# stochasticHydroTools/PSE

Measured on AMD Instinct MI355X. Metric: BD particle-steps/s (full PSE Brownian step: M.F + k-space noise + Lanczos M^1/2.psi + Euler), N=1e6, phi=0.1, higher is better.
Workload: dtype f64; 1 GPU; random-sphere suspension N=1000000, phi=0.1, cubic L=347.29, grid 256^3, xi=0.4405, rcut=5.966, P=6, error=0.001, kT=1.0, dt=0.001; parallelism=1 GPU

## Files before the change

pse_amd/csrc/pse_capi.hip:

```cpp
#include <hip/hip_runtime.h>
#include <rccl/rccl.h>
#include <rocfft/rocfft.h>

#include <algorithm>
#include <chrono>
#include <cmath>
#include <cstdarg>
#include <cstdio>
#include <cstring>
#include <dlfcn.h>
#include <functional>
#include <future>
#include <memory>
#include <mutex>
#include <thread>
#include <string>
#include <vector>

#include "../../include/pse_amd.h"
#include "pse_err.h"
#include "pse_host.h"
#include "pse_kernels.h"
#include "pse_farfield.h"
#include "pse_fft.h"
// ... 637 lines not shown
        if (T->m[0]->grid_slabs > 1) *mask |= 1u << PH_COMM;
        TRY(wave_compute(*T, a, 0));
        next = 1;
        if (T->m[0]->grid_slabs == 1) return upto(1 << 30);
        return 0;
    }
    int upto(int e) {
        while (T && next <= 3 && slot[next - 1] <= e) {
            TRY(wave_exchange(*T, next - 1));
            TRY(wave_compute(*T, a, next));
            ++next;
        }
        return 0;
    }
    int drain() { return upto(1 << 30); }
};

static int row_ranges(const pse_handle *h, int N, int depth, int rg[3][2]) {
    if (h->n_slabs == 1) { rg[0][0] = 0; rg[0][1] = N; return 1; }
    const int G = h->n_slabs, r = h->slab_rank, L = (r + G - 1) % G, R = (r + 1) % G;
    int n = 0;
    auto add = [&](int a, int b) {
        if (b <= a) return;
        for (int q = 0; q < n; ++q) if (rg[q][0] == a && rg[q][1] == b) return;
        rg[n][0] = a; rg[n][1] = b; ++n;
    };
    rg[0][0] = h->row_lo[r]; rg[0][1] = h->row_lo[r + 1]; n = 1;
    if (depth >= 1) {
        add((depth == 1 ? h->last_begin : h->last2_begin)[L], h->row_lo[L + 1]);
        add(h->row_lo[R], (depth == 1 ? h->first_end : h->first2_end)[R]);
    }
    return n;
}
static RowMap rank_rows(const pse_handle *h, int N, int depth) {
    int rg[3][2];
    const int n = row_ranges(h, N, depth, rg);
    return row_map(rg, n);
}

static int real(pse_team &T, double4 *pse_handle::*vec, double4 *pse_handle::*out, size_t vec_off, size_t out_off, int N,
                bool build_list, bool with_psi = false, int depth = 0) {
    for (pse_handle *h : act(T)) {
        h->w_is_mpsi = false;
        int mode = MREAL_CELLS;
        if (h->nb.cap > 0) {
            if (h->nb_valid) mode = MREAL_USE_LIST;
            else if (build_list) mode = MREAL_BUILD_LIST;
        }
        int vlm = VL_NONE;
        if (h->vl_use) vlm = VL_USE;
        else if (h->vl_pending && mode != MREAL_USE_LIST) vlm = VL_WRITE;
        const double4 *v = h->*vec + vec_off;
        if (h->gated && mode == MREAL_CELLS) {
            const RowMap rows = rank_rows(h, N, 0);
            const int nco = h->n_intervals * 2 * RS_NCOEF;
            const Gate rb{h->gate_word, 1}, ru{h->gate_word, 0};
            launch_mreal(h->pos_s, h->posf_s, v, h->*out + out_off, rows, h->cell_off, h->dbox, h->nc, h->d.rcut, h->d.self, h->coef, nco,
                         h->nb, MREAL_CELLS, h->stream, nullptr, nullptr, h->vl, VL_WRITE, nullptr, nullptr, 0, nullptr, rb);
            launch_gate_copy(rb, h->pos_build, h->pos_s, (size_t)N, h->stream);
            launch_mreal(h->pos_s, h->posf_s, v, h->*out + out_off, rows, h->cell_off, h->dbox, h->nc, h->d.rcut, h->d.self, h->coef, nco,
                         h->nb, MREAL_CELLS, h->stream, nullptr, nullptr, h->vl, VL_USE,
                         v == h->f_s && h->pv_is_f ? h->pv : nullptr, nullptr, 0, nullptr, ru);
            h->vl_valid = true; h->vl_box = h->box;
            continue;
        }
        const bool psi = with_psi && mode == MREAL_BUILD_LIST;
        launch_mreal(h->pos_s, h->posf_s, v, h->*out + out_off, rank_rows(h, N, mode == MREAL_BUILD_LIST ? depth : 0), h->cell_off, h->dbox,
                     h->nc, h->d.rcut, h->d.self, h->coef, h->n_intervals * 2 * RS_NCOEF, h->nb, mode, h->stream,
                     psi ? h->psi_s : nullptr, h->w_s, h->vl, vlm,
                     v == h->f_s && h->pv_is_f && (vlm == VL_USE || mode != MREAL_USE_LIST) ? h->pv : nullptr,
                     psi && h->n_slabs == 1 ? h->partials : nullptr, h->npart_cap, h->scal);
        h->sums0_done = psi && h->n_slabs == 1 && vlm != VL_USE && mreal_table_in_lds(h->n_intervals * 2 * RS_NCOEF);
        if (vlm == VL_WRITE) {
            HIPCHK(hipMemcpyAsync(h->pos_build, h->pos_s, (size_t)N * sizeof(double4), hipMemcpyDeviceToDevice, h->stream));
            h->vl_pending = false; h->vl_valid = true; h->vl_box = h->box;
        }
        if (mode == MREAL_BUILD_LIST) { h->nb_valid = true; h->w_is_mpsi = with_psi && (vlm == VL_USE || mreal_table_in_lds(h->n_intervals * 2 * RS_NCOEF)); }
    }
    return 0;
}

static int update_ranges(const pse_handle *h, int N, int rg[3][2]) { return row_ranges(h, N, 1, rg); }

static double4 *lz_vec(const pse_handle *h, int q) { return q < 0 ? nullptr : q == 0 ? h->psi_s : h->V + (size_t)q * h->n_pad; }
static LzBlockArgs lz_block_args(const pse_handle *h, int j, bool full) {
    LzBlockArgs a{};
    a.q = lz_vec(h, j); a.p = lz_vec(h, j - 1); a.w1 = h->w_s; a.w2 = full ? h->w2_s : nullptr;
    a.u = h->u_s; a.v1 = lz_vec(h, j + 1); a.v2 = full ? lz_vec(h, j + 2) : nullptr;
    a.j = j;
    return a;
}
static int lz_m_in(const int *m_io) { return std::min(std::max(m_io ? *m_io : 2, 1), M_MAX); }
static int lz_queued_extra(const pse_handle *h, int m_in) {
    return std::max(0, std::min(h->lz_extra >= 0 ? h->lz_extra : h->tun.lz_extra, M_MAX - std::max(m_in, 2)));
}

static int lz_wait_scalars(pse_team &T, bool &hook_done, const std::function<int()> &before_first_wait) {
    pse_handle *h0 = T.m[0];
    HIPCHK(hipEventRecord(h0->ev_scal, h0->stream));
    if (!hook_done) {
        hook_done = true;
        for (pse_handle *h : act(T)) TRY(te(h, PH_LANCZOS));
        if (before_first_wait) TRY(before_first_wait());
    }
    HIPCHK(hipEventSynchronize(h0->ev_scal));
    return 0;
}
static int lz_decide_batch(LzDecide d, int m_in, int done, double tol, const double *sc, LzState &st) {
    d.m_lo = std::max((d.first ? 0 : st.checked) + 1, std::max(m_in - 1, 1)); d.m_hi = d.done_iters = done; d.m_max = M_MAX; d.tol = tol;
    int at = 0;
    const LzFailure f = lz_decide_host(d, sc, st, &at);
    if (f == LZ_NONFINITE) return fail(PSE_ERR_NUMERIC, "Lanczos produced a non-finite coefficient at iteration %d", at);
    if (f == LZ_EIGEN_FAILED) return fail(PSE_ERR_NUMERIC, "tridiagonal eigen-solve failed at m = %d", at);
    return 0;
}
static int lz_zero_result(pse_team &T, int N, int matvecs) {
    for (pse_handle *h : act(T)) {
        HIPCHK(hipMemsetAsync(h->ub_s, 0, (size_t)N * sizeof(double4), h->stream));
        h->info.lanczos_m = 0; h->info.lanczos_matvecs = matvecs; h->info.lanczos_stepnorm = 0.0;
    }
    return 0;
}
static void lz_combine(pse_team &T, int N, double scale, const LzState &st, int matvecs, int exchanges) {
    BasisCoef tc{};
    std::copy(st.coef, st.coef + st.m_final, tc.t);
    for (pse_handle *h : act(T)) {
        int lo, hi;
        row_range(h, N, lo, hi);
        launch_basis_combine(h->psi_s, h->V, h->n_pad, tc, st.m_final, h->scal, scale, 1, h->ub_s, lo, hi, h->stream, h->sink);
        h->tail_done = h->sink.on;
        h->info.lanczos_m = st.m_final; h->info.lanczos_matvecs = matvecs; h->info.lanczos_stepnorm = st.stepnorm;
        h->info.lanczos_exchanges = exchanges;
    }
}

static int lanczos_queued(pse_team &T, int N, double tol, double scale, int *m_io, const std::function<int()> &before_first_wait,
                          const std::function<int()> &before_combine) {
    pse_handle *h = T.m[0];
    const int m_in = lz_m_in(m_io), target = std::max(m_in, 2), extra = lz_queued_extra(h, m_in);
    const int *stop = &h->lz_state->done;
    const double seq = (double)++h->lz_seq;
    h->lz_last_queued = true;
    int rg[3][2];
    const int nrg_all = update_ranges(h, N, rg);
    auto vector_part = [&](int j, const int *gate) {
        launch_lz_update(lz_vec(h, j), h->w_s, lz_vec(h, j - 1), lz_vec(h, j + 1), j, h->scal, rg, nrg_all, h->stream,
                         nullptr, 0, h->sc_host_dev, gate, vq_of(h), h->lz_sums);
    };
    auto iteration = [&](int j, bool scalars_only, const int *gate) -> int {
        const bool have_y = j == 0 && h->w_is_mpsi;
        const bool fused = !have_y && h->nb.cap > 0 && h->nb_valid;
        if (!fused && !have_y) {
            if (gate) return fail(PSE_ERR_NUMERIC, "queued Lanczos: a gated iteration needs the pair list");
            TRY(real(T, j == 0 ? &pse_handle::psi_s : &pse_handle::V, &pse_handle::w_s, (size_t)j * h->n_pad, 0, N, true));
        }
        const double4 *vjm1 = lz_vec(h, j - 1);
        const bool split = fused && j > 0;
        if (fused)
            launch_mreal_lanczos(h->pos_s, lz_vec(h, j), h->w_s, row_map(0, N), h->cell_off, h->dbox, h->nc, h->d.rcut, h->d.self, h->coef, h->nb,
                                 LzFuse{split ? nullptr : vjm1, h->partials, h->npart_cap, nullptr, nullptr, nullptr, h->lz_sums, lz_update_grid(N)}, h->scal, nullptr, nullptr, h->stream,
                                 h->vl_use ? h->vl : VerletList{}, split ? 4 : 1, gate, DevRowArgs{}, j > 0 ? vq_of(h) : nullptr);
        else if (!(j == 0 && h->sums0_done))
            launch_lz_dots(lz_vec(h, j), h->w_s, vjm1, 0, N, h->partials, h->npart_cap, h->scal, h->stream);
        h->w_is_mpsi = false; h->sums0_done = false;
        if (scalars_only) launch_lz_update(lz_vec(h, j), h->w_s, vjm1, lz_vec(h, j + 1), j, h->scal, rg, 0, h->stream, nullptr, 0,
                                           h->sc_host_dev, gate);
        else vector_part(j, gate);
        return 0;
    };
    for (int j = 0; j < target; ++j) TRY(iteration(j, j == target - 1, nullptr));
    LzDecide d{};
    d.m_lo = std::max(m_in - 1, 1); d.m_hi = target; d.done_iters = target; d.first = 1; d.last = extra == 0 ? 1 : 0; d.m_max = M_MAX; d.tol = tol;
    launch_lz_decide(d, h->scal, h->lz_state, h->sc_host_dev, seq, h->stream);
    int done = target;
    for (int x = 0; x < extra; ++x) {
        vector_part(done - 1, stop);
        TRY(iteration(done, true, stop));
        d.m_lo = d.m_hi = done + 1; d.done_iters = done + 1; d.pending_beta = done; d.first = 0; d.last = x == extra - 1 ? 1 : 0;
        launch_lz_decide(d, h->scal, h->lz_state, h->sc_host_dev, seq, h->stream);
        ++done;
    }
    TRY(te(h, PH_LANCZOS));
    if (before_first_wait) TRY(before_first_wait());
    if (before_combine) TRY(before_combine());
    launch_basis_combine(h->psi_s, h->V, h->n_pad, BasisCoef{}, 0, h->scal, scale, 1, h->ub_s, 0, N, h->stream, h->sink, h->lz_state);
    h->tail_done = h->sink.on;
    h->info.lanczos_matvecs = done; h->info.lanczos_exchanges = 0;
    if (m_io) *m_io = h->sc_host[LZ_HOST_SEQ] > 0.0 && h->sc_host[LZ_HOST_M] >= 1.0 ? (int)h->sc_host[LZ_HOST_M] : m_in;
    HIPCHK(hipGetLastError());
    return 0;
}

static int lanczos(pse_team &T, int N, double tol, double scale, int *m_io, const std::function<int()> &before_first_wait = nullptr,
                   WavePump *pump = nullptr, const std::function<int()> &before_combine = nullptr) {
    pse_handle *h0 = T.m[0];
    const int m_in = lz_m_in(m_io);
    if (h0->async_mode && T.G == 1 && T.solo < 0 && h0->nb.cap > 0 && !h0->timing &&
        lz_decide_supported(std::max(m_in, 2) + lz_queued_extra(h0, m_in)))
        return lanczos_queued(T, N, tol, scale, m_io, before_first_wait, before_combine);
    for (pse_handle *h : act(T)) h->lz_last_queued = false;
    const double *sc = h0->sc_host;
    int done = 0, n_exchanges = 0;
    int target = std::max(m_in, 2);
    int pending_beta = 0;
    LzState st{0, 0, 0, 0, 1.0, {}, {}};
    bool hook_done = false;
    auto update = [&](int j, bool scalars_only) {
        for (pse_handle *h : act(T)) {
            int rg[3][2];
            const int nrg = scalars_only ? 0 : update_ranges(h, N, rg);
            launch_lz_update(lz_vec(h, j), h->w_s, lz_vec(h, j - 1), lz_vec(h, j + 1), j, h->scal, rg, nrg, h->stream, h->sums_all, T.G > 1 ? T.G : 0,
                             h == h0 ? h->sc_host_dev : nullptr, nullptr, T.G <= 1 ? vq_of(h) : nullptr, T.G <= 1 ? h->lz_sums : nullptr);
        }
    };
    while (true) {
        for (; done < target; ++done) {
            const bool have_y = done == 0 && h0->w_is_mpsi;
            const bool fused = !have_y && h0->nb.cap > 0 && h0->nb_valid;
            const bool timed = done == 1 && fused;
            if (!fused && !have_y) TRY(real(T, done == 0 ? &pse_handle::psi_s : &pse_handle::V, &pse_handle::w_s, (size_t)done * h0->n_pad, 0, N, true));
            for (pse_handle *h : act(T)) {
                int lo, hi;
                row_range(h, N, lo, hi);
                const double4 *xj = lz_vec(h, done), *vjm1 = lz_vec(h, done - 1);
                if (fused) {
                    const bool ev = timed && h->timing;
                    const bool split = done > 0 && T.G <= 1;
                    launch_mreal_lanczos(h->pos_s, xj, h->w_s, row_map(lo, hi), h->cell_off, h->dbox, h->nc, h->d.rcut, h->d.self, h->coef,
                                         h->nb, LzFuse{split ? nullptr : vjm1, h->partials, h->npart_cap, nullptr, nullptr, nullptr, h->lz_sums, lz_update_grid(N)}, h->scal,
                                         ev ? h->ph[PH_MATVEC].a : nullptr, ev ? h->ph[PH_MATVEC].b : nullptr, h->stream,
                                         h->vl_use ? h->vl : VerletList{}, split ? 4 : 1, nullptr, DevRowArgs{}, done > 0 && T.G <= 1 ? vq_of(h) : nullptr);
                    if (timed) h->matvec_timed = true;
                } else if (!(done == 0 && h->sums0_done)) {
                    launch_lz_dots(xj, h->w_s, vjm1, lo, hi, h->partials, h->npart_cap, h->scal, h->stream);
                }
                h->w_is_mpsi = false; h->sums0_done = false;
            }
            if (pump) TRY(pump->upto(n_exchanges));
            ++n_exchanges;
            TRY(team_lanczos_exchange(T, [](pse_handle *h) { return (double *)h->w_s; }));
            update(done, done == target - 1);
        }
        TRY(lz_wait_scalars(T, hook_done, before_first_wait));
        if (T.solo >= 0) { st.m_final = done; break; }
        LzDecide d{};
        d.first = pending_beta == 0; d.pending_beta = pending_beta;
        TRY(lz_decide_batch(d, m_in, done, tol, sc, st));
        if (st.done) break;
        update(done - 1, false);
        pending_beta = done;
        target = std::min(M_MAX, done + std::max(2, done / 4));
    }
    if (st.m_final == 0) {
        if (m_io) *m_io = m_in;
        return lz_zero_result(T, N, done);
    }
    if (before_combine) TRY(before_combine());
    lz_combine(T, N, scale, st, done, T.G > 1 ? n_exchanges : 0);
    if (m_io) *m_io = st.m_final;
    return 0;
}

static int lanczos_team(pse_team &T, int N, double tol, double scale, int *m_io, const std::function<int()> &before_first_wait,
                        WavePump *pump, const std::function<int()> &before_combine = nullptr) {
    pse_handle *h0 = T.m[0];
    for (pse_handle *h : act(T)) h->lz_last_queued = false;
    const int m_in = lz_m_in(m_io);
    const double *sc = h0->sc_host;
    int done = 0, target = std::max(m_in, 2), n_exchanges = 0, matvecs = 0;
    int half_pending = -1;
    bool first = true;
    LzState st{0, 0, 0, 0, 1.0, {}, {}};
    bool hook_done = false;
    while (true) {
        while (done < target) {
            if (half_pending >= 0) {
                for (pse_handle *h : act(T)) {
                    int rg[3][2];
                    const int nrg = row_ranges(h, N, 2, rg);
                    launch_lz_block(lz_block_args(h, half_pending, false), false, h->scal, rg, nrg, h->stream, h->sums_all, T.G, h == h0 ? h->sc_host_dev : nullptr);
                }
                half_pending = -1;
            }
            const int j = done;
            const bool full = target - done >= 2 && j + 2 <= M_MAX;
            for (pse_handle *h : act(T)) {
                const LzFuse lz{nullptr, h->partials, h->npart_cap, lz_vec(h, j), lz_vec(h, j - 1), j > 0 ? h->u_s : nullptr};
                if (j == 0 && !h->w_is_mpsi) return fail(PSE_ERR_NUMERIC, "two-step Lanczos: M psi did not come with the pair list");
                if (!(j == 0 && h->w_is_mpsi)) {
                    launch_mreal_lanczos(h->pos_s, lz_vec(h, j), h->w_s, rank_rows(h, N, full ? 1 : 0), h->cell_off, h->dbox, h->nc, h->d.rcut,
                                         h->d.self, h->coef, h->nb, lz, h->scal, nullptr, nullptr, h->stream, VerletList{}, full ? 0 : 3);
                    ++matvecs;
                } else if (!full) {
                    return fail(PSE_ERR_NUMERIC, "two-step Lanczos: a single step cannot start at j = 0");
                }
                h->w_is_mpsi = false;
                if (full) {
                    launch_mreal_lanczos(h->pos_s, h->w_s, h->w2_s, rank_rows(h, N, 0), h->cell_off, h->dbox, h->nc, h->d.rcut, h->d.self,
                                         h->coef, h->nb, lz, h->scal, nullptr, nullptr, h->stream, VerletList{}, 2);
                    ++matvecs;
                }
            }
            if (pump) TRY(pump->upto(n_exchanges));
            ++n_exchanges;
            TRY(team_run_exchange(T, [&](pse_handle *h) {
                                      auto ops = ghost_ops(h, T.G, {(double *)h->w_s, full ? (double *)h->w2_s : nullptr}, 2);
                                      sum_ops(h, T.G, LZ_NGRAM, ops);
                                      return ops; },
                                  false, DIAG_LANCZOS));
            for (pse_handle *h : act(T)) {
                int rg[3][2];
                const int nrg = full ? row_ranges(h, N, 2, rg) : 0;
                launch_lz_block(lz_block_args(h, j, full), full, h->scal, rg, nrg, h->stream, h->sums_all, T.G, h == h0 ? h->sc_host_dev : nullptr);
            }
            if (full) done += 2; else { done += 1; half_pending = j; }
        }
        TRY(lz_wait_scalars(T, hook_done, before_first_wait));
        if (T.solo >= 0) { st.m_final = done; break; }
        LzDecide d{};
        d.first = first; d.have_last_beta = d.normalised = 1;
        TRY(lz_decide_batch(d, m_in, done, tol, sc, st));
        if (st.done) break;
        first = false;
        target = std::min(M_MAX, done + std::max(2, done / 4));
    }
    if (st.m_final == 0) {
        if (m_io) *m_io = m_in;
        return lz_zero_result(T, N, matvecs);
    }
    if (half_pending >= 0 && st.m_final > half_pending + 1) return fail(PSE_ERR_NUMERIC, "two-step Lanczos: basis vector %d was never formed", half_pending + 1);
    if (before_combine) TRY(before_combine());
    lz_combine(T, N, scale, st, matvecs, n_exchanges);
    if (m_io) *m_io = st.m_final;
    return 0;
}

struct Args {
    const double4 *pos; const double4 *force; double4 *vel;
};

struct StepArgs {
    double4 *pos; double4 *vel; double3 *accel; int3 *image; const double4 *force;
};
struct StepTail { const std::vector<StepArgs> *sa; double dt, shear_rate; };

static int velocity(pse_team &T, const std::vector<Args> &a, const unsigned *group, int N, int parts, double kT, double dt,
                    unsigned timestep, int *m_io, unsigned *mask, const StepTail *tail = nullptr) {
    for (pse_handle *h : T.m)
        if (h->loc.on) return fail(PSE_ERR_INVALID, "this handle is an owned-particle rank (pse_params.local_rows): drive it through pse_team_step_local");
    for (pse_handle *h : T.m) h->tail_done = false;
    diag_begin(T);
    for (size_t r = 0; r < T.m.size(); ++r)
        if (T.solo < 0 || T.m[r]->slab_rank == T.solo)
            TRY(prepare(T.m[r], a[r].pos, a[r].force, group, N, true, false, PrepExtra{kT > 0.0, timestep}, (parts & 1) != 0));
    *mask |= 1u << PH_SORT;
    const bool noise = kT > 0.0;
    const bool sstep = T.G > 1 && noise && (parts & 1) && team_sstep(T.m[0]);
    for (pse_handle *h : act(T)) {
        const bool on = h->side && parts == 3 && !h->timing && (T.G > 1 ? T.lanes : (h->overlap_all || !noise));
        if (on != h->side_on || h->wstream != (on ? h->side : h->stream)) {
            h->side_on = on;
            h->wstream = on ? h->side : h->stream;
            TRY(bind_wave_stream(h));
        }
    }
    WavePump pump;
    const WaveArgs wa{N, noise, kT, dt, timestep};
    auto wave_start = [&]() -> int { return pump.start(T, wa, T.m[0]->tun.team_sched, mask); };
    const bool wave_behind = noise && (parts & 2) && (parts & 1) && !T.m[0]->side_on;
    const bool near_first = noise && parts == 3 && T.m[0]->side_on;
// ... 74 lines not shown
        }
        HIPCHK(hipGetLastError());
    }
    diag_mark(T, 1, act(T)[0]->stream);
    return 0;
}

static int team_of_one(pse_handle *h, pse_team &T) {
    if (h->n_slabs > 1) return fail(PSE_ERR_INVALID, "this handle is a slab rank: drive it through a pse_team");
    T.m = {h}; T.G = 1;
    return 0;
}

static int do_mobility(pse_team &T, const std::vector<Args> &a, const unsigned *group, unsigned N, int parts) {
    for (pse_handle *h : T.m) TRY(check_n(h, N));
    for (auto &x : a) if (!x.pos || !x.force || !x.vel) return fail(PSE_ERR_INVALID, "null array");
    if (!(parts & 3)) return fail(PSE_ERR_INVALID, "parts must select real (1), wave (2) or both (3)");
    unsigned mask = 1u << PH_TOTAL;
    for (pse_handle *h : act(T)) TRY(ts(h, PH_TOTAL));
    TRY(velocity(T, a, group, (int)N, parts, 0.0, 1.0, 0, nullptr, &mask));
    for (pse_handle *h : act(T)) { TRY(te(h, PH_TOTAL)); TRY(collect_times(h, mask)); }
    return 0;
}

static int do_brownian(pse_team &T, const std::vector<Args> &a, const unsigned *group, unsigned N, double kT, double dt,
                       unsigned timestep, int *lanczos_m, int parts = 3) {
    for (pse_handle *h : act(T)) TRY(check_n(h, N));
    for (auto &x : a) if (!x.pos || !x.force || !x.vel) return fail(PSE_ERR_INVALID, "null array");
    if (kT < 0 || !(dt > 0)) return fail(PSE_ERR_INVALID, "need kT >= 0 and dt > 0");
    unsigned mask = 1u << PH_TOTAL;
    for (pse_handle *h : act(T)) TRY(ts(h, PH_TOTAL));
    TRY(velocity(T, a, group, (int)N, parts, kT, dt, timestep, lanczos_m, &mask));
    for (pse_handle *h : act(T)) { TRY(te(h, PH_TOTAL)); TRY(collect_times(h, mask)); }
    return 0;
}

static int do_step(pse_team &T, const std::vector<StepArgs> &sa, const unsigned *group, unsigned N, double kT, double dt,
                   unsigned timestep, double shear_rate, int *lanczos_m) {
    for (pse_handle *h : act(T)) TRY(check_n(h, N));
    std::vector<Args> a;
    for (auto &x : sa) {
        if (!x.pos || !x.vel || !x.accel || !x.image || !x.force) return fail(PSE_ERR_INVALID, "null array");
        a.push_back(Args{x.pos, x.force, x.vel});
    }
    if (kT < 0 || !(dt > 0)) return fail(PSE_ERR_INVALID, "need kT >= 0 and dt > 0");
    unsigned mask = (1u << PH_TOTAL) | (1u << PH_INTEG);
    for (pse_handle *h : act(T)) TRY(ts(h, PH_TOTAL));
    for (pse_handle *h : act(T)) h->vl_kind = 1;
    const StepTail tail{&sa, dt, shear_rate};
    const int rc_v = velocity(T, a, group, (int)N, 3, kT, dt, timestep, lanczos_m, &mask, &tail);
    for (pse_handle *h : act(T)) h->vl_kind = 0;
    if (rc_v) return rc_v;
    for (pse_handle *h : act(T)) {
        TRY(te(h, PH_TOTAL));
        HIPCHK(hipGetLastError());
        TRY(collect_times(h, mask));
    }
    return 0;
}

static LocalRegions local_regions(const pse_handle *h) {
    const LocalGeom &g = h->loc.g;
    const int lc = layer_cells(h->nc), nx = g.nx;
    auto wrap = [&](int l) { return ((l % nx) + nx) % nx; };
    LocalRegions r{};
    const int l_own = g.rank * g.per, l_gl = wrap(l_own - g.depth), l_gr = wrap(l_own + g.per);
    r.c0[0] = l_own * lc; r.c1[0] = (l_own + g.per) * lc; r.base[0] = 0; r.cap[0] = g.c_own;
    r.c0[1] = l_gl * lc; r.c1[1] = (l_gl + g.depth) * lc; r.base[1] = g.c_own; r.cap[1] = g.c_g;
    r.c0[2] = l_gr * lc; r.c1[2] = (l_gr + g.depth) * lc; r.base[2] = g.c_own + g.c_g; r.cap[2] = g.c_g;
    r.c_first_end = (l_own + g.depth) * lc - 1;
    r.c_last_begin = (l_own + g.per - g.depth) * lc;
    r.c_gl_adj = wrap(l_own - 1) * lc;
    r.c_gr_adj = (l_gr + 1) * lc - 1;
    return r;
}

static int lanczos_local(pse_team &T, double tol, int *m_io, WavePump *pump) {
    pse_handle *h0 = T.m[0];
    const int m_in = lz_m_in(m_io), target = std::max(m_in, 2);
    const int extra_blocks = ((T.lz_extra >= 0 ? T.lz_extra : h0->tun.lz_extra) + 1) / 2;
    if (target + 2 * extra_blocks > M_MAX || !lz_decide_supported(target + 2 * extra_blocks))
        return fail(PSE_ERR_INVALID, "owned-particle step: starting count %d of the Lanczos iteration is beyond what the device-side decision takes", m_in);
    int n_exchanges = 0, matvecs = 0, done = 0, half_pending = -1;
    auto fuse = [&](pse_handle *h, int j) { return LzFuse{nullptr, h->partials, h->npart_cap, lz_vec(h, j), lz_vec(h, j - 1), j > 0 ? h->u_s : nullptr}; };
    auto exchange = [&](bool full) -> int {
        if (pump) TRY(pump->upto(n_exchanges));
        ++n_exchanges;
        return team_run_exchange(T, [&](pse_handle *h) {
            const LocalGeom &g = h->loc.g;
            const int L = (g.rank + g.G - 1) % g.G, R = (g.rank + 1) % g.G;
            const size_t cnt = (size_t)g.c_g * 4;
            std::vector<Xfer> ops;
            ops.push_back(Xfer{(double *)h->w_s, cnt, L, (double *)(h->w_s + g.c_own + g.c_g), cnt, R});
            ops.push_back(Xfer{(double *)h->loc.stage_w1, cnt, R, (double *)(h->w_s + g.c_own), cnt, L});
            if (full) {
                ops.push_back(Xfer{(double *)h->w2_s, cnt, L, (double *)(h->w2_s + g.c_own + g.c_g), cnt, R});
                ops.push_back(Xfer{(double *)h->loc.stage_w2, cnt, R, (double *)(h->w2_s + g.c_own), cnt, L});
            }
            sum_ops(h, T.G, LZ_NGRAM, ops);
            return ops; }, false, DIAG_LANCZOS);
    };
    auto full_block = [&](int j, bool gated) -> int {
        for (pse_handle *h : act(T)) {
            const int *gate = gated ? &h->lz_state->done : nullptr;
            const LocalRows *R = h->loc.rows;
            if (j == 0) {
                if (!h->w_is_mpsi) return fail(PSE_ERR_NUMERIC, "owned-particle step: M psi did not come with the pair list");
            } else {
                launch_mreal_lanczos(h->pos_s, lz_vec(h, j), h->w_s, RowMap{}, h->cell_off, h->dbox, h->nc, h->d.rcut, h->d.self, h->coef, h->nb, fuse(h, j),
                                     h->scal, nullptr, nullptr, h->stream, VerletList{}, 0, gate,
                                     DevRowArgs{&R->own1, R, h->loc.stage_w1, h->loc.rows_cap, h->loc.g.c_g});
                ++matvecs;
            }
            h->w_is_mpsi = false;
            launch_mreal_lanczos(h->pos_s, h->w_s, h->w2_s, RowMap{}, h->cell_off, h->dbox, h->nc, h->d.rcut, h->d.self, h->coef, h->nb, fuse(h, j), h->scal,
                                 nullptr, nullptr, h->stream, VerletList{}, 2, gate, DevRowArgs{&R->own, R, h->loc.stage_w2, h->loc.g.c_own, h->loc.g.c_g});
            ++matvecs;
        }
        TRY(exchange(true));
        for (pse_handle *h : act(T))
            launch_lz_block(lz_block_args(h, j, true), true, h->scal, nullptr, 0, h->stream, h->sums_all, T.G, h->sc_host_dev, &h->loc.rows->all,
                            h->loc.rows_cap, false, gated ? &h->lz_state->done : nullptr);
        return 0;
    };
    auto single = [&](int j, bool gated) -> int {
        for (pse_handle *h : act(T)) {
            const LocalRows *R = h->loc.rows;
            launch_mreal_lanczos(h->pos_s, lz_vec(h, j), h->w_s, RowMap{}, h->cell_off, h->dbox, h->nc, h->d.rcut, h->d.self, h->coef, h->nb, fuse(h, j), h->scal,
                                 nullptr, nullptr, h->stream, VerletList{}, 3, gated ? &h->lz_state->done : nullptr,
                                 DevRowArgs{&R->own, R, h->loc.stage_w1, h->loc.g.c_own, h->loc.g.c_g});
            ++matvecs;
        }
        TRY(exchange(false));
        for (pse_handle *h : act(T))
            launch_lz_block(lz_block_args(h, j, false), false, h->scal, nullptr, 0, h->stream, h->sums_all, T.G, h->sc_host_dev, &h->loc.rows->all,
                            h->loc.rows_cap, true, gated ? &h->lz_state->done : nullptr);
        half_pending = j;
        return 0;
    };
    auto decide = [&](int m_lo, int m_hi, int done_iters, bool first, bool last) {
        for (pse_handle *h : act(T)) {
            LzDecide d{};
            d.m_lo = m_lo; d.m_hi = m_hi; d.done_iters = done_iters; d.have_last_beta = 1; d.first = first ? 1 : 0; d.last = last ? 1 : 0;
            d.normalised = 1; d.m_max = M_MAX; d.tol = T.solo >= 0 ? 1e300 : tol;
            launch_lz_decide(d, h->scal, h->lz_state, h->sc_host_dev, (double)h->lz_seq, h->stream);
        }
    };
    for (pse_handle *h : act(T)) { ++h->lz_seq; h->lz_last_queued = true; }
    while (target - done >= 2) { TRY(full_block(done, false)); done += 2; }
    if (target - done == 1) { TRY(single(done, false)); done += 1; }
    decide(std::max(m_in - 1, 1), target, done, true, extra_blocks == 0);
    for (int x = 0; x < extra_blocks; ++x) {
        if (half_pending >= 0) {
            for (pse_handle *h : act(T))
                launch_lz_block(lz_block_args(h, half_pending, false), false, h->scal, nullptr, 0, h->stream, h->sums_all, T.G, h->sc_host_dev,
                                &h->loc.rows->all, h->loc.rows_cap, false, &h->lz_state->done);
            half_pending = -1;
        }
        TRY(full_block(done, true));
        decide(done + 1, done + 2, done + 2, false, x == extra_blocks - 1);
        done += 2;
    }
    for (pse_handle *h : act(T)) { h->info.lanczos_matvecs = matvecs; h->info.lanczos_exchanges = n_exchanges; }
    if (m_io) *m_io = !remote(T) && h0->sc_host[LZ_HOST_SEQ] > 0.0 && h0->sc_host[LZ_HOST_M] >= 1.0 ? (int)h0->sc_host[LZ_HOST_M] : m_in;
    return 0;
}

// ... 140 lines not shown
    if (parts < 1 || parts > 3) return fail(PSE_ERR_INVALID, "parts must select real (1), wave (2) or both (3)");
    if (!pos || !force || !vel) return fail(PSE_ERR_INVALID, "null array");
    pse_team T;
    TRY(team_of_one(h, T));
    return do_brownian(T, {Args{(const double4 *)pos, (const double4 *)force, (double4 *)vel}}, group, N, kT, dt, timestep, lanczos_m, parts);
}

extern "C" int pse_integrate(pse_handle *h, pse_double4 *pos, const pse_double4 *vel, pse_double3 *accel, pse_int3 *image,
                             const pse_double4 *net_force, const unsigned *group, unsigned N, double dt, double shear_rate) {
    if (!h) return fail(PSE_ERR_INVALID, "null handle");
    if (!pos || !vel || !accel || !image || !net_force) return fail(PSE_ERR_INVALID, "null array");
    if (!(dt > 0)) return fail(PSE_ERR_INVALID, "need dt > 0");
    TRY(check_n(h, N));
    HIPCHK(hipSetDevice(h->device));
    launch_integrate((double4 *)pos, (const double4 *)vel, (double3 *)accel, (int3 *)image, (const double4 *)net_force, group, (int)N, h->dbox, dt,
                     shear_rate, h->stream);
    HIPCHK(hipGetLastError());
    return 0;
}

extern "C" int pse_step(pse_handle *h, pse_double4 *pos, pse_double4 *vel, pse_double3 *accel, pse_int3 *image,
                        const pse_double4 *net_force, const unsigned *group, unsigned N, double kT, double dt,
                        unsigned timestep, double shear_rate, int *lanczos_m) {
    if (!h) return fail(PSE_ERR_INVALID, "null handle");
    pse_team T;
    TRY(team_of_one(h, T));
    return do_step(T, {StepArgs{(double4 *)pos, (double4 *)vel, (double3 *)accel, (int3 *)image, (const double4 *)net_force}},
                   group, N, kT, dt, timestep, shear_rate, lanczos_m);
}

extern "C" int pse_sqrt_mreal(pse_handle *h, const pse_double4 *pos, const pse_double4 *psi, pse_double4 *out,
                              const unsigned *group, unsigned N, double tol, int *lanczos_m) {
    TRY(check_n(h, N));
    if (!pos || !psi || !out) return fail(PSE_ERR_INVALID, "null array");
    pse_team T;
    TRY(team_of_one(h, T));
    TRY(prepare(h, (const double4 *)pos, (const double4 *)psi, group, (int)N));
    HIPCHK(hipMemcpyAsync(h->psi_s, h->f_s, (size_t)N * sizeof(double4), hipMemcpyDeviceToDevice, h->stream));
    TRY(lanczos(T, (int)N, tol, 1.0, lanczos_m));
    launch_scatter_sum(h->ub_s, nullptr, nullptr, h->tag_s, (int)N, (double4 *)out, h->stream);
    HIPCHK(hipGetLastError());
    return 0;
}

extern "C" int pse_random_psi(pse_handle *h, pse_double4 *psi, const unsigned *group, unsigned N, unsigned timestep) {
    TRY(check_n(h, N));
    if (!psi) return fail(PSE_ERR_INVALID, "null array");
    std::vector<unsigned> tags(N);
    if (group) HIPCHK(hipMemcpy(tags.data(), group, N * sizeof(unsigned), hipMemcpyDeviceToHost));
    else for (unsigned i = 0; i < N; ++i) tags[i] = i;
    HIPCHK(hipMemcpy(h->tag_s, tags.data(), N * sizeof(unsigned), hipMemcpyHostToDevice));
    launch_psi(h->psi_s, h->tag_s, (int)N, h->par.seed, timestep, h->stream);
    launch_scatter_sum(h->psi_s, nullptr, nullptr, h->tag_s, (int)N, (double4 *)psi, h->stream);
    HIPCHK(hipStreamSynchronize(h->stream));
    h->sorted_N = 0;
    return 0;
}

extern "C" int pse_eval_realspace(pse_handle *h, const double *r_host, int n, double *f_host, double *g_host) {
    if (!h || !r_host || !f_host || !g_host || n <= 0) return fail(PSE_ERR_INVALID, "bad argument");
    HIPCHK(hipSetDevice(h->device));
    for (int i = 0; i < n; ++i)
        if (!(r_host[i] > 0.0) || r_host[i] * RS_PER_UNIT * (1.0 + 0x1p-50) >= h->n_intervals)
            return fail(PSE_ERR_INVALID, "r[%d] = %g outside the table range (0, %g)", i, r_host[i], (double)h->n_intervals / RS_PER_UNIT);
    double *buf = nullptr;
    HIPCHK(hipMalloc((void **)&buf, (size_t)3 * n * sizeof(double)));
    hipError_t e = hipMemcpy(buf, r_host, n * sizeof(double), hipMemcpyHostToDevice);
    if (e == hipSuccess) {
        launch_eval_fg(buf, n, h->coef, buf + n, buf + 2 * n, h->stream);
        e = hipStreamSynchronize(h->stream);
    }
    if (e == hipSuccess) e = hipMemcpy(f_host, buf + n, n * sizeof(double), hipMemcpyDeviceToHost);
    if (e == hipSuccess) e = hipMemcpy(g_host, buf + 2 * n, n * sizeof(double), hipMemcpyDeviceToHost);
    (void)hipFree(buf);
    if (e != hipSuccess) return fail(PSE_ERR_HIP, "pse_eval_realspace: %s", hipGetErrorString(e));
    return 0;
}

extern "C" int pse_debug_matvec_ms(pse_handle *h, int reps, float *ms_per_launch) {
    if (!h || !ms_per_launch || reps < 1) return fail(PSE_ERR_INVALID, "pse_debug_matvec_ms: bad argument");
    HIPCHK(hipSetDevice(h->device));
    if (h->n_slabs != 1 || !h->nb_valid || h->nb.cap <= 0 || h->sorted_N <= 0)
        return fail(PSE_ERR_INVALID, "pse_debug_matvec_ms: needs the pair list of a Brownian call on a single-GPU engine (call it right after one)");
    const size_t stride = h->n_pad;
    const int N = h->sorted_N;
    RowMap rm{};
    rm.n = 1; rm.lo[0] = 0; rm.hi[0] = N;
    hipEvent_t e0 = nullptr, e1 = nullptr;
    HIPCHK(hipEventCreate(&e0)); HIPCHK(hipEventCreate(&e1));
    auto run = [&](int n) {
        for (int r = 0; r < n; ++r)
            launch_mreal_lanczos(h->pos_s, h->V + stride, h->w_s, rm, h->cell_off, h->dbox, h->nc, h->d.rcut, h->d.self, h->coef, h->nb,
                                 LzFuse{h->psi_s, h->partials, h->npart_cap, nullptr, nullptr, nullptr}, h->scal, nullptr, nullptr, h->stream,
                                 VerletList{}, 1, nullptr, DevRowArgs{}, vq_of(h), true);
    };
    run(2);
    HIPCHK(hipEventRecord(e0, h->stream));
    run(reps);
    HIPCHK(hipEventRecord(e1, h->stream));
    HIPCHK(hipEventSynchronize(e1));
    float ms = 0;
    HIPCHK(hipEventElapsedTime(&ms, e0, e1));
    (void)hipEventDestroy(e0); (void)hipEventDestroy(e1);
    HIPCHK(hipGetLastError());
    *ms_per_launch = ms / (float)reps;
    return 0;
}
extern "C" int pse_debug_vq_roundtrip(int n, const double *rows_host, double *out_host) {
    if (n < 0 || (n > 0 && (!rows_host || !out_host))) return fail(PSE_ERR_INVALID, "pse_debug_vq_roundtrip: null argument");
    if (n == 0) return 0;
    double *d_in = nullptr, *d_out = nullptr;
    hipError_t e = hipMalloc((void **)&d_in, (size_t)3 * n * sizeof(double));
    if (e == hipSuccess) e = hipMalloc((void **)&d_out, (size_t)3 * n * sizeof(double));
    if (e == hipSuccess) e = hipMemcpy(d_in, rows_host, (size_t)3 * n * sizeof(double), hipMemcpyHostToDevice);
    if (e == hipSuccess) { launch_vq_roundtrip(d_in, d_out, n, nullptr); e = hipGetLastError(); }
    if (e == hipSuccess) e = hipMemcpy(out_host, d_out, (size_t)3 * n * sizeof(double), hipMemcpyDeviceToHost);
    (void)hipFree(d_in); (void)hipFree(d_out);
    if (e != hipSuccess) return fail(PSE_ERR_HIP, "pse_debug_vq_roundtrip: %s", hipGetErrorString(e));
    return 0;
}
static_assert(PSE_DEBUG_LZ_NSCAL == LZ_NSCAL && LZ_HOST_OPEN == LZ_HOST_M + 4 && LZ_HOST_OPEN < LZ_NSCAL, "pse_debug_lz_decide: layout of the scalars");
extern "C" int pse_debug_lz_decide_supported(int m_hi) { return lz_decide_supported(m_hi) ? 1 : 0; }
extern "C" int pse_debug_lz_decide(const double *scal_host, int n_dec, const pse_debug_lz_decision *dec, double open0, pse_debug_lz_outcome *out) {
    if (int rc = lz_decisions_validate("pse_debug_lz_decide", scal_host, n_dec, dec, out)) return rc;
    for (int k = 0; k < n_dec; ++k) {
        const pse_debug_lz_decision &d = dec[k];
        if (!lz_decide_supported(d.m_hi)) return fail(PSE_ERR_INVALID, "pse_debug_lz_decide: decision %d: m_hi = %d is not supported", k, d.m_hi);
        if (d.m_lo < d.m_hi - 1)
            return fail(PSE_ERR_INVALID, "pse_debug_lz_decide: decision %d: m_lo = %d is not m_hi or m_hi - 1 (m_hi = %d)", k, d.m_lo, d.m_hi);
    }
    double *scal = nullptr, *sch = nullptr;
    LzState *st = nullptr;
    std::vector<double> mirror(LZ_NSCAL, 0.0);
    mirror[LZ_HOST_OPEN] = open0;
    hipError_t e = hipMalloc((void **)&scal, LZ_NSCAL * sizeof(double));
    if (e == hipSuccess) e = hipMalloc((void **)&sch, LZ_NSCAL * sizeof(double));
    if (e == hipSuccess) e = hipMalloc((void **)&st, sizeof(LzState));
    if (e == hipSuccess) e = hipMemcpy(scal, scal_host, LZ_NSCAL * sizeof(double), hipMemcpyHostToDevice);
    if (e == hipSuccess) e = hipMemcpy(sch, mirror.data(), LZ_NSCAL * sizeof(double), hipMemcpyHostToDevice);
    if (e == hipSuccess) e = hipMemset(st, 0xff, sizeof(LzState));
    for (int k = 0; k < n_dec && e == hipSuccess; ++k) {
        launch_lz_decide(lz_decision(dec[k]), scal, st, sch, dec[k].seq, nullptr);
        e = hipGetLastError();
        LzState hs;
        if (e == hipSuccess) e = hipMemcpy(&hs, st, sizeof(LzState), hipMemcpyDeviceToHost);
        if (e == hipSuccess) e = hipMemcpy(out[k].mirror, sch + LZ_HOST_M, 5 * sizeof(double), hipMemcpyDeviceToHost);
        if (e != hipSuccess) break;
        lz_outcome(hs, &out[k]);
    }
    (void)hipFree(scal); (void)hipFree(sch); (void)hipFree(st);
    if (e != hipSuccess) return fail(PSE_ERR_HIP, "pse_debug_lz_decide: %s", hipGetErrorString(e));
    return 0;
}
extern "C" int pse_debug_grid_placement(pse_handle *h, int *tried, float *ms_first, float *ms_kept) {
    if (!h || !tried || !ms_first || !ms_kept) return fail(PSE_ERR_INVALID, "pse_debug_grid_placement: null argument");
    *tried = h->place_tried; *ms_first = h->place_ms_first; *ms_kept = h->place_ms_kept;
    return 0;
}
extern "C" int pse_debug_kvector(pse_handle *h, int n, const int *ijk_host, double *out_host) {
    if (!h || !ijk_host || !out_host || n <= 0) return fail(PSE_ERR_INVALID, "bad argument");
    HIPCHK(hipSetDevice(h->device));
    for (int t = 0; t < n; ++t)
        if (ijk_host[3 * t] < 0 || ijk_host[3 * t] >= h->G.Nx || ijk_host[3 * t + 1] < 0 || ijk_host[3 * t + 1] >= h->G.Ny ||
            ijk_host[3 * t + 2] < 0 || ijk_host[3 * t + 2] >= h->G.Nz)
            return fail(PSE_ERR_INVALID, "node %d outside the %d x %d x %d grid", t, h->G.Nx, h->G.Ny, h->G.Nz);
    int *d_ijk = nullptr;
    double *d_out = nullptr;
    HIPCHK(hipMalloc((void **)&d_ijk, (size_t)3 * n * sizeof(int)));
    hipError_t e = hipMalloc((void **)&d_out, (size_t)5 * n * sizeof(double));
    if (e == hipSuccess) e = hipMemcpy(d_ijk, ijk_host, (size_t)3 * n * sizeof(int), hipMemcpyHostToDevice);
    if (e == hipSuccess) {
        launch_debug_kop(d_ijk, n, h->G, h->dbox, h->d.xi, h->d.eta, d_out, h->stream);
        e = hipStreamSynchronize(h->stream);
    }
    if (e == hipSuccess) e = hipMemcpy(out_host, d_out, (size_t)5 * n * sizeof(double), hipMemcpyDeviceToHost);
// ... 448 lines not shown
```

pse_amd/csrc/pse_device.h:

```cpp
#pragma once
#include <hip/hip_runtime.h>
#include <stdint.h>
#include <atomic>

#include "pse_host.h"

namespace pse {

struct DBox {
    double Lx, Ly, Lz, xy;
    double iLx, iLy, iLz;
};

struct DGrid {
    int Nx, Ny, Nz, Nzh;
    int Nzp;
    int P;
    int x0, nxl;
    int nhalo;
    int hl;
    double hx, hy, hz;
    double prefac, expfac;
};

struct DCells {
    int nx, ny, nz;
    int bz, nzb;
    int xpad;
};
__host__ __device__ inline int layer_cells(const DCells &nc) { return nc.nzb * nc.ny * nc.bz + nc.xpad; }
__host__ __device__ inline int cells_total(const DCells &nc) { return nc.nx * layer_cells(nc); }
__host__ __device__ inline int cell_slot(const DCells &nc, int cx, int cy, int zb, int zi) { return ((cx * nc.nzb + zb) * nc.ny + cy) * nc.bz + zi + cx * nc.xpad; }

__device__ __forceinline__ void frac_coords(const DBox &b, double x, double y, double z, double &fx, double &fy, double &fz) {
    fx = (x - b.xy * y) * b.iLx + 0.5;
    fy = y * b.iLy + 0.5;
    fz = z * b.iLz + 0.5;
    fx -= floor(fx); fy -= floor(fy); fz -= floor(fz);
    if (fx >= 1.0) fx = 0.0;
    if (fy >= 1.0) fy = 0.0;
    if (fz >= 1.0) fz = 0.0;
}

__device__ __forceinline__ void min_image(const DBox &b, double &dx, double &dy, double &dz) {
    const double ny = rint(dy * b.iLy);
    dy -= ny * b.Ly;
    dx -= ny * b.xy * b.Ly;
    dx -= rint(dx * b.iLx) * b.Lx;
    dz -= rint(dz * b.iLz) * b.Lz;
}

__device__ __forceinline__ int cell_coord(double f, int n) {
    int c = (int)(f * n);
    c = c < 0 ? 0 : c;
    return c >= n ? n - 1 : c;
}

__device__ __forceinline__ int xcd_block(int b, int nb) {
    const int q = nb >> 3, r = nb & 7, x = b & 7, k = b >> 3;
    return (x < r ? x * (q + 1) : r * (q + 1) + (x - r) * q) + k;
}

typedef unsigned vq4 __attribute__((ext_vector_type(4)));
__device__ __forceinline__ vq4 vq_pack(double x, double y, double z) {
    const double m = fmax(fabs(x), fmax(fabs(y), fabs(z)));
    int e = 0;
    (void)frexp(m, &e);
    e = e < -100 ? -100 : (e > 127 ? 127 : e);
    const double sc = __hiloint2double((39 - e + 1023) << 20, 0);
    const double lim = 549755813887.0;
    const long long ix = (long long)fmax(-lim, fmin(lim, rint(x * sc))), iy = (long long)fmax(-lim, fmin(lim, rint(y * sc))),
                    iz = (long long)fmax(-lim, fmin(lim, rint(z * sc)));
    vq4 w;
    w.x = (unsigned)ix; w.y = (unsigned)iy; w.z = (unsigned)iz;
    w.w = ((unsigned)(ix >> 32) & 0xffu) | (((unsigned)(iy >> 32) & 0xffu) << 8) | (((unsigned)(iz >> 32) & 0xffu) << 16) | ((unsigned)(e + 128) << 24);
    return w;
}
__device__ __forceinline__ void vq_unpack(vq4 w, double &x, double &y, double &z) {
    const int e = (int)(w.w >> 24) - 128;
    const double sc = __hiloint2double((e - 39 + 1023) << 20, 0);
    const int hx = (int)(w.w << 24) >> 24, hy = (int)(w.w << 16) >> 24, hz = (int)(w.w << 8) >> 24;
    x = fma((double)hx, 4294967296.0, (double)w.x) * sc;
    y = fma((double)hy, 4294967296.0, (double)w.y) * sc;
    z = fma((double)hz, 4294967296.0, (double)w.z) * sc;
}

constexpr int TPB = 256;
static inline int nblocks(long n, int tpb) { return (int)((n + tpb - 1) / tpb); }
__device__ __forceinline__ double wave_sum(double v) {
#pragma unroll
    for (int o = 32; o > 0; o >>= 1) v += __shfl_xor(v, o, 64);
    return v;
}
__device__ __forceinline__ double block_sum(double v, double *sh ) {
    v = wave_sum(v);
    const int w = threadIdx.x >> 6;
    __syncthreads();
    if ((threadIdx.x & 63) == 0) sh[w] = v;
    __syncthreads();
    return sh[0] + sh[1] + sh[2] + sh[3];
}
__device__ __forceinline__ double reduce_partials(const double *partials, int n, double *sh) {
    double v = 0.0;
    for (int i = threadIdx.x; i < n; i += TPB) v += partials[i];
    return block_sum(v, sh);
}
struct LdsAttr {
    std::atomic<size_t> have[32];
    bool need(size_t lds) {
        int dev = 0;
        (void)hipGetDevice(&dev);
        if (dev < 0 || dev >= 32) return true;
        if (have[dev].load(std::memory_order_relaxed) >= lds) return false;
        have[dev].store(lds, std::memory_order_relaxed);
        return true;
    }
};
template <auto K, class... Args>
static void launch_lds(dim3 grid, dim3 block, size_t lds, hipStream_t s, Args... args) {
    static LdsAttr attr;
    if (attr.need(lds)) (void)hipFuncSetAttribute(reinterpret_cast<const void *>(K), hipFuncAttributeMaxDynamicSharedMemorySize, (int)lds);
    hipLaunchKernelGGL(K, grid, block, lds, s, args...);
}

__device__ __forceinline__ int wrapi(int a, int n) { a %= n; return a < 0 ? a + n : a; }

constexpr uint32_t PHILOX_KEY1 = 0x50534531u;
constexpr uint32_t DOMAIN_PARTICLE = 0, DOMAIN_GRID_A = 1, DOMAIN_GRID_B = 2;

__host__ __device__ __forceinline__ void philox4x32(uint32_t c0, uint32_t c1, uint32_t c2, uint32_t c3,
                                                    uint32_t k0, uint32_t k1, uint32_t out[4]) {
#pragma unroll
    for (int r = 0; r < 10; ++r) {
        const uint64_t p0 = (uint64_t)0xD2511F53u * c0, p1 = (uint64_t)0xCD9E8D57u * c2;
        const uint32_t n0 = (uint32_t)(p1 >> 32) ^ c1 ^ k0, n1 = (uint32_t)p1;
        const uint32_t n2 = (uint32_t)(p0 >> 32) ^ c3 ^ k1, n3 = (uint32_t)p0;
        c0 = n0; c1 = n1; c2 = n2; c3 = n3;
        k0 += 0x9E3779B9u; k1 += 0xBB67AE85u;
    }
    out[0] = c0; out[1] = c1; out[2] = c2; out[3] = c3;
}

__host__ __device__ __forceinline__ double uniform_pm(uint32_t x, double s) {
    return (((double)x + 0.5) * 2.3283064365386963e-10 * 2.0 - 1.0) * s;
}

__device__ __forceinline__ double exp_lean(double x) {
    const double n = rint(x * 1.4426950408889634074);
    double r = fma(n, -6.93147180369123816490e-01, x);
    r = fma(n, -1.90821492927058770002e-10, r);
    double p = 1.6059043836821613e-10;
    p = fma(p, r, 2.08767569878681e-09);
    p = fma(p, r, 2.505210838544172e-08);
    p = fma(p, r, 2.755731922398589e-07);
    p = fma(p, r, 2.7557319223985893e-06);
    p = fma(p, r, 2.48015873015873e-05);
    p = fma(p, r, 1.984126984126984e-04);
    p = fma(p, r, 1.388888888888889e-03);
    p = fma(p, r, 8.333333333333333e-03);
    p = fma(p, r, 4.1666666666666664e-02);
    p = fma(p, r, 1.6666666666666666e-01);
    p = fma(p, r, 0.5);
    p = fma(p, r, 1.0);
    p = fma(p, r, 1.0);
    return ldexp(p, (int)n);
}
__device__ __forceinline__ double exp_neg(double x) { return exp_lean(x); }

__device__ __forceinline__ double sin_lean(double x) {
    const double n = rint(x * 0.31830988618379067154);
    double r = fma(-n, 3.14159265358979311600, x);
    r = fma(-n, 1.2246467991473531772e-16, r);
    const double r2 = r * r;
    double p = -1.9572941063391261231e-20;
    p = fma(p, r2, 8.2206352466243297170e-18);
    p = fma(p, r2, -2.8114572543455207632e-15);
    p = fma(p, r2, 7.6471637318198164759e-13);
    p = fma(p, r2, -1.6059043836821614599e-10);
    p = fma(p, r2, 2.5052108385441718775e-08);
    p = fma(p, r2, -2.7557319223985890653e-06);
    p = fma(p, r2, 1.9841269841269841270e-04);
    p = fma(p, r2, -8.3333333333333333333e-03);
    p = fma(p, r2, 1.6666666666666666667e-01);
// ... 92 lines not shown
```

pse_amd/csrc/pse_engine.hip:

```cpp
#include <hip/hip_runtime.h>
#include <rocfft/rocfft.h>

#include <algorithm>
#include <cmath>
#include <cstdio>
#include <cstring>
#include <mutex>
#include <string>
#include <vector>

#include "pse_forces.h"
#include "pse_handle.h"

static std::once_flag g_fft_once;

static int set_lanczos_op(pse_handle *h, int op) {
    if (op == PSE_LANCZOS_FP64 && h->nb.cap > 0 && !h->nb64) {
        HIPCHK(hipSetDevice(h->device));
        TRY(dmalloc(h, &h->nb64, nb_list64_bytes((size_t)h->n_pad + 1024, h->nb.cap) / sizeof(double4)));
        h->info.device_bytes = h->bytes;
    }
    if (op != h->lz_op) h->nb_valid = false;
    h->lz_op = op;
    h->nb.c64 = op == PSE_LANCZOS_FP64 ? h->nb64 : nullptr;
// ... 151 lines not shown
                                                       dims, cs, cdist, dims, rs, rdist));
        FFTCHK(h->fft.plan(&h->plan_fwd, rocfft_placement_notinplace, rocfft_transform_type_real_forward, dims, len, batch, df));
        FFTCHK(h->fft.plan(&h->plan_inv, rocfft_placement_notinplace, rocfft_transform_type_real_inverse, dims, len, batch, di));
        rocfft_plan_description_destroy(df);
        rocfft_plan_description_destroy(di);
        return 0;
    };
    if (h->own_y) {
        const size_t len1[1] = {(size_t)G.Nz};
        TRY(real_plans(1, len1, (size_t)3 * G.Nx * G.Ny));
    } else if (h->xfuse && h->grid_slabs == 1) {
        const size_t len2[2] = {(size_t)G.Nz, (size_t)G.Ny};
        TRY(real_plans(2, len2, (size_t)3 * G.Nx));
    } else if (h->grid_slabs == 1) {
        const size_t len[3] = {(size_t)G.Nz, (size_t)G.Ny, (size_t)G.Nx};
        TRY(real_plans(3, len, 3));
    } else {
        const size_t len2[2] = {(size_t)G.Nz, (size_t)G.Ny};
        const size_t len1[1] = {(size_t)G.Nz};
        if (h->own_y_slab) TRY(real_plans(1, len1, (size_t)G.nxl * G.Ny));
        else TRY(real_plans(2, len2, (size_t)G.nxl));
        const size_t lenx[1] = {(size_t)G.Nx};
        size_t stride[1] = {(size_t)h->nyl * G.Nzp};
        rocfft_plan_description desc = nullptr;
        FFTCHK(rocfft_plan_description_create(&desc));
        FFTCHK(rocfft_plan_description_set_data_layout(desc, rocfft_array_type_complex_interleaved,
                                                       rocfft_array_type_complex_interleaved, nullptr, nullptr, 1, stride, 1,
                                                       1, stride, 1));
        FFTCHK(h->fft.plan(&h->plan_x_fwd, rocfft_placement_inplace, rocfft_transform_type_complex_forward, 1, lenx, stride[0], desc));
        FFTCHK(h->fft.plan(&h->plan_x_inv, rocfft_placement_inplace, rocfft_transform_type_complex_inverse, 1, lenx, stride[0], desc));
        rocfft_plan_description_destroy(desc);
        FFTCHK(rocfft_plan_get_work_buffer_size(h->plan_x_fwd, &w)); work = std::max(work, w);
        FFTCHK(rocfft_plan_get_work_buffer_size(h->plan_x_inv, &w)); work = std::max(work, w);
    }
    FFTCHK(rocfft_plan_get_work_buffer_size(h->plan_fwd, &w)); work = std::max(work, w);
    FFTCHK(rocfft_plan_get_work_buffer_size(h->plan_inv, &w)); work = std::max(work, w);
    h->fft_work_bytes = work;
    if (work) TRY(dmalloc(h, (char **)&h->fft_work, work));
    FFTCHK(h->fft.info(&h->info_fwd));
    FFTCHK(h->fft.info(&h->info_inv));
    if (work) {
        FFTCHK(rocfft_execution_info_set_work_buffer(h->info_fwd, h->fft_work, work));
        FFTCHK(rocfft_execution_info_set_work_buffer(h->info_inv, h->fft_work, work));
    }
    return bind_wave_stream(h);
}

static int create_impl(const pse_params *p, pse_handle *h) {
    h->par = *p;
    h->box = Box{p->Lx, p->Ly, p->Lz, p->xy};
    std::string e = select_params(h->box, p->xi, p->error, p->max_strain, p->Nx, p->Ny, p->Nz, p->P, p->rcut, h->d);
    if (!e.empty()) return fail(PSE_ERR_INVALID, "%s", e.c_str());
    if (p->n_max == 0) return fail(PSE_ERR_INVALID, "n_max must be positive");
    TRY(gaussian_fits(h->d, h->d.hx, h->d.hy, h->d.hz));
    if (!(std::fabs(p->xy) <= 0.5 * (1.0 + 1e-9)))
        return fail(PSE_ERR_INVALID, "tilt xy = %g outside [-0.5, 0.5]: HOOMD flips the box there, and the sequential minimum image "
                    "(PSEv1/Mobility.cu:648) is exact only up to that tilt", p->xy);
    const Derived &d = h->d;
    if (p->device >= 0) { HIPCHK(hipSetDevice(p->device)); h->device = p->device; }
    else HIPCHK(hipGetDevice(&h->device));
    h->n_max = (int)p->n_max;
    set_dbox(h);
    h->n_slabs = std::max(1, p->n_slabs);
    h->loc.on = p->local_rows != 0;
    if (h->loc.on && h->n_slabs < 2) return fail(PSE_ERR_INVALID, "local_rows needs n_slabs >= 2 (an owned-particle rank is a member of a team)");
    roctx_lookup();
    {
        auto ienv = [](const char *name, int dflt) { const char *v = getenv(name); return v ? atoi(v) : dflt; };
        auto &t = h->tun;
        t.cell_bz = std::min(16, std::max(0, ienv("PSE_CELL_BZ", 6)));
        if (const char *v = getenv("PSE_SKIN")) t.skin = atof(v);
        t.overlap = ienv("PSE_OVERLAP", 1);
        t.no_xfuse = getenv("PSE_NO_XFUSE") != nullptr;
        t.own_y = ienv("PSE_OWN_Y", 1); t.own_y_pow2 = ienv("PSE_OWN_Y_POW2", 1); t.yfft_kb = ienv("PSE_YFFT_KB", 4); t.own_z = ienv("PSE_OWN_Z", 1); t.yslab_regs = ienv("PSE_YSLAB_REGS", 1);
        if (const char *v = getenv("PSE_WAVE_MODE")) t.wave_mode = !strcmp(v, "slab") ? 1 : (!strcmp(v, "replicated") ? 2 : 0);
        t.spread_tz = ienv("PSE_SPREAD_TZ", 0); t.spread_nw = ienv("PSE_SPREAD_NW", 0);
        t.gather_bz = ienv("PSE_GATHER_BZ", 0); t.xmix_runtime = ienv("PSE_XMIX", 0) == 1; t.xfft_small_wide = ienv("PSE_XFFT_SMALL_KB", 2) == 8;
        t.verbose = ienv("PSE_VERBOSE", 0) > 0;
        t.team_sstep = ienv("PSE_TEAM_SSTEP", 1) > 0;
        t.lz_extra = std::max(0, std::min(32, ienv("PSE_LANCZOS_EXTRA", 2)));
        t.place_trials = std::max(0, std::min(12, ienv("PSE_PLACE_TRIALS", 10)));
        t.vq = ienv("PSE_VQ", 1);
        if (const char *v = getenv("PSE_LANCZOS_OP")) t.lz_op = !strcmp(v, "fp64") ? PSE_LANCZOS_FP64 : PSE_LANCZOS_RECORDS16;
        if (const char *v = getenv("PSE_TEAM_SCHED")) {
            int a = 1, b = 2, c = 3;
            if (sscanf(v, "%d,%d,%d", &a, &b, &c) == 3) { t.team_sched[0] = a; t.team_sched[1] = b; t.team_sched[2] = c; }
        }
        h->sw.force_tz = t.spread_tz; h->sw.force_nw = t.spread_nw; h->sw.force_bz = t.gather_bz;
    }
    {
        double skin = h->tun.skin;
        const int nint = (int)std::ceil(d.rcut * RS_PER_UNIT) + 1;
        const double gam = std::max(std::fabs(p->xy), p->max_strain);
        const double wmin = std::min(std::min(h->box.Lx / std::sqrt(1.0 + gam * gam), h->box.Ly), h->box.Lz);
        if (!(skin > 0.0) || h->n_slabs > 1 || !mreal_table_in_lds(nint * 2 * RS_NCOEF) || d.rcut + skin > 0.5 * wmin)
            skin = 0.0;
        h->skin = h->skin_max = skin;
    }
    TRY(set_cells(h, std::max(std::fabs(p->xy), p->max_strain)));
    fill_info(d, &h->info);
    h->info.ncell_x = h->nc.nx; h->info.ncell_y = h->nc.ny; h->info.ncell_z = h->nc.nz;

    DGrid &G = h->G;
    G.Nx = d.Nx; G.Ny = d.Ny; G.Nz = d.Nz; G.Nzh = d.Nz / 2 + 1; G.P = d.P;
    G.Nzp = (G.Nzh + 7) & ~7;
    h->n_slabs = std::max(1, p->n_slabs);
    h->slab_rank = h->n_slabs > 1 ? p->slab_rank : 0;
    if (h->slab_rank < 0 || h->slab_rank >= h->n_slabs) return fail(PSE_ERR_INVALID, "slab_rank outside [0, n_slabs)");
    h->grid_slabs = h->n_slabs;
    if (h->n_slabs > 1) {
        const bool replicate = h->tun.wave_mode ? h->tun.wave_mode == 2 : h->n_slabs == 2;
        if (replicate && !h->loc.on) h->grid_slabs = 1;
    }
    if (h->grid_slabs > 1) {
        if (d.Nx % h->grid_slabs || d.Ny % h->grid_slabs)
            return fail(PSE_ERR_INVALID, "slab decomposition needs Nx and Ny divisible by the number of ranks (%d x %d over %d)",
                        d.Nx, d.Ny, h->grid_slabs);
        if (d.Nx / h->grid_slabs < d.P)
            return fail(PSE_ERR_INVALID, "slabs of %d planes are thinner than the support P = %d", d.Nx / h->grid_slabs, d.P);
    }
    const int grid_rank = h->grid_slabs > 1 ? h->slab_rank : 0;
    G.nxl = d.Nx / h->grid_slabs; G.x0 = grid_rank * G.nxl;
    G.hl = h->grid_slabs > 1 ? (d.P - 1) / 2 : 0;
    G.nhalo = h->grid_slabs > 1 ? (d.P + 1) / 2 : 0;
    h->nyl = d.Ny / h->grid_slabs; h->y0 = grid_rank * h->nyl;
    G.hx = d.hx; G.hy = d.hy; G.hz = d.hz;
    const double c = 2.0 * d.xi * d.xi / d.eta;
    G.expfac = c;
    G.prefac = (c / M_PI) * std::sqrt(c / M_PI);

    const size_t n = ((size_t)h->n_max + h->n_slabs - 1) / h->n_slabs * h->n_slabs;
    h->n_pad = (int)n;
    TRY(dmalloc(h, &h->keys, n)); TRY(dmalloc(h, &h->keys_s, n)); TRY(dmalloc(h, &h->vals, n));
    TRY(dmalloc(h, &h->perm, n)); TRY(dmalloc(h, &h->tag_s, n));

    {
        const double rc = d.rcut;
        auto cnt = [&](double w) { int c2 = (int)std::floor(w / rc); if (c2 < 3) c2 = 1; if (c2 > 1024) c2 = 1024; return (size_t)c2; };
        h->n_cells_alloc = cnt(h->box.Lx) * cnt(h->box.Ly) * (cnt(h->box.Lz) + 16) + cnt(h->box.Lx);
    }
    TRY(dmalloc(h, &h->cell_off, h->n_cells_alloc + 1));
    h->sort_tmp_bytes = cell_sort_temp_bytes(h->n_cells_alloc);
    TRY(dmalloc(h, (char **)&h->sort_tmp, h->sort_tmp_bytes));
    const size_t nbins = (size_t)((d.Nx + 7) / 8) * ((d.Ny + 7) / 8) * ((d.Nz + 7) / 8);
    const bool fast_far = d.P >= 4 && d.P <= FAR_PMAX;
    h->cnt_bins = ((fast_far ? nbins + 1 : 0) + 1 + 3) & ~(size_t)3;
    constexpr size_t LAYER_INTS = (size_t)LOCAL_MAX_LAYERS * LOCAL_LAYER_SLOTS;
    TRY(dmalloc(h, &h->cnt_block, h->cnt_bins + 4 + h->n_cells_alloc + 1 + 8 + LOCAL_NCOUNTER + 2 + LAYER_INTS + 4));
    h->loc.counters = h->cnt_block + ((h->cnt_bins + 4 + h->n_cells_alloc + 1 + 8 + 1) & ~(size_t)1);
    h->loc.layer_cnt = h->loc.counters + LOCAL_NCOUNTER;
    h->loc.zero_ints = ((size_t)(h->loc.layer_cnt - h->cnt_block) + LAYER_INTS + 3) & ~(size_t)3;
    if (h->nc.nx > LOCAL_MAX_LAYERS && p->local_rows) return fail(PSE_ERR_INVALID, "more than %d cell layers along x", LOCAL_MAX_LAYERS);
    h->vl.flags = h->cnt_block + h->cnt_bins - 1;
    h->gate_word = h->cnt_block + h->cnt_bins + 1;
    h->cell_cnt = h->cnt_block + h->cnt_bins + 4;
    if (fast_far) {
        h->sw.fb.cnt = h->cnt_block;
        TRY(dmalloc(h, (char **)&h->sw.rec_t, (n + 64) * 64));
        TRY(dmalloc(h, &h->sw.fb.rank_s, n));
        TRY(dmalloc(h, &h->sw.fb.off, nbins + 1));
        h->sw.fb.tmp_bytes = bin_scan_temp_bytes(nbins);
        TRY(dmalloc(h, (char **)&h->sw.fb.tmp, h->sw.fb.tmp_bytes));
    }
    std::vector<double> coef;
    build_realspace_table(d.xi, d.rcut, coef, h->n_intervals);
    TRY(dmalloc(h, &h->coef, coef.size()));
// ... 8 lines not shown
        const double bytes = (double)cap * (double)n * 20.0;
        if (bytes > 32e9 || n >= ((size_t)1 << 27)) cap = 0;
        h->nb.cap = cap;
        if (cap > 0) {
            TRY(dmalloc(h, &h->nb.data, nb_list_bytes(n + 1024, cap)));
        }
        if (cap == 0) h->skin = h->skin_max = 0.0;
        if (h->skin_max > 0.0) {
            const double rs = d.rcut + h->skin_max, nbar_v = n_box / vol * 4.18879020478639 * rs * rs * rs;
            h->vl.cap = (std::max(16, std::min((int)std::ceil(2.0 * nbar_v + 32.0), 512)) + 3) & ~3;
            h->vl.rskin = rs;
            TRY(dmalloc(h, (char **)&h->vl.idx, verlet_list_bytes(n + 1024, h->vl.cap)));
            TRY(dmalloc(h, &h->vl.cnt, n));
            TRY(dmalloc(h, &h->pos_build, n));
            HIPCHK(h->pinned.make((void **)&h->flags_host, 2 * sizeof(int)));
        }
    }
    TRY(dmalloc(h, &h->pos_s, n)); TRY(dmalloc(h, &h->posf_s, n));
    TRY(dmalloc(h, &h->pv, 3 * n));
    TRY(dmalloc(h, &h->f_s, n)); TRY(dmalloc(h, &h->uw_s, n)); TRY(dmalloc(h, &h->ur_s, n));
    TRY(dmalloc(h, &h->ub_s, n)); TRY(dmalloc(h, &h->psi_s, n)); TRY(dmalloc(h, &h->w_s, n));

    const size_t nr = (size_t)(G.nxl + G.hl + G.nhalo) * G.Ny * G.Nz, ncx = (size_t)G.nxl * G.Ny * G.Nzp;
    TRY(dmalloc(h, &h->rgrid, 3 * nr));
    TRY(dmalloc(h, &h->cgrid, 3 * ncx));
    if (h->grid_slabs > 1) { TRY(dmalloc(h, &h->sendbuf, 3 * ncx)); TRY(dmalloc(h, &h->recvbuf, 3 * ncx)); }
    if (h->n_slabs > 1) {
        HIPCHK(h->pinned.make((void **)&h->bounds_host, ((size_t)5 * h->n_slabs + 1) * sizeof(int), hipHostMallocMapped));
        HIPCHK(hipHostGetDevicePointer((void **)&h->bounds_host_dev, h->bounds_host, 0));
        HIPCHK(h->events.make(&h->ev_bounds, hipEventDisableTiming));
        TRY(dmalloc(h, &h->d_bidx, (size_t)5 * h->n_slabs + 1)); TRY(dmalloc(h, &h->d_bounds, (size_t)5 * h->n_slabs + 1));
        TRY(dmalloc(h, &h->utot_s, n));
        TRY(dmalloc(h, &h->sums_all, (size_t)h->n_slabs * LZ_NGRAM));
        if (h->tun.team_sstep && h->nb.cap > 0) {
            TRY(dmalloc(h, &h->w2_s, n)); TRY(dmalloc(h, &h->u_s, n));
        }
    }
    if (h->loc.on) {
        auto &L = h->loc;
        const int G_ = h->n_slabs, per = h->nc.nx / G_, depth = 2;
        if (per < depth + 1 || (G_ - 1) * per < 2 * depth)
            return fail(PSE_ERR_INVALID, "an owned-particle rank needs >= %d cell layers of width rcut per rank along x (%d ranks: %d layers each)",
                        G_ == 2 ? 2 * depth : depth + 1, G_, per);
        if (!team_sstep(h))
            return fail(PSE_ERR_INVALID, "an owned-particle rank needs the per-step pair list and the real-space table in LDS (rcut = %.3f, n_max = %d)",
                        d.rcut, h->n_max);
        if ((d.P / 2 + 1.0) / d.Nx > (double)depth / h->nc.nx)
            return fail(PSE_ERR_INVALID, "the spreading support (P = %d on %d planes) reaches beyond the %d ghost cell layers of an owned-particle rank", d.P, d.Nx, depth);
        const int c_g = (int)((double)h->n_max * depth / (per + 2 * depth)) / 256 * 256, c_own = (h->n_max - 2 * c_g) / 256 * 256;
        if (c_g < 256 || c_own < c_g)
            return fail(PSE_ERR_INVALID, "n_max = %d is too small a row capacity for an owned-particle rank (%d layers + 2 x %d ghost layers)", h->n_max, per, depth);
        L.g = LocalGeom{h->slab_rank, G_, per, depth, h->nc.nx, c_own, c_g, c_g};
        L.rows_cap = c_own + 2 * c_g;
        L.msg = (size_t)LOCAL_HDR + (size_t)LOCAL_REC * c_g;
        for (int q = 0; q < 2; ++q) { TRY(dmalloc(h, &L.send[q], L.msg)); TRY(dmalloc(h, &L.recv[q], L.msg)); HIPCHK(hipMemset(L.recv[q], 0, L.msg * sizeof(double))); }
        TRY(dmalloc(h, &L.stage_w1, (size_t)c_g)); TRY(dmalloc(h, &L.stage_w2, (size_t)c_g));
        TRY(dmalloc(h, &L.porig_s, (size_t)c_own)); TRY(dmalloc(h, &L.mass_s, (size_t)c_own)); TRY(dmalloc(h, &L.image_s, (size_t)c_own));
        TRY(dmalloc(h, &L.rows, 1));
        TRY(dmalloc(h, &L.err, 4));
        HIPCHK(hipMemset(L.err, 0, 4 * sizeof(int)));
        HIPCHK(hipMemset(L.rows, 0, sizeof(LocalRows)));
        HIPCHK(h->pinned.make((void **)&L.err_host, 4 * sizeof(int)));
        L.err_host[0] = 0;
    }
    h->wstream = h->stream;
    if (h->tun.overlap >= 0) {
        {
            int lo = 0, hi = 0;
            (void)hipDeviceGetStreamPriorityRange(&lo, &hi);
            const char *pr = getenv("PSE_SIDE_PRIORITY");
            if (!pr || !*pr) pr = h->loc.on ? "low" : "default";
            const int prio = !strcmp(pr, "low") ? lo : hi;
            HIPCHK(h->streams.make(&h->side, hipStreamNonBlocking, !strcmp(pr, "low") || !strcmp(pr, "high") ? &prio : nullptr));
        }
        h->side_owned = h->side;
        HIPCHK(h->events.make(&h->ev_fork, hipEventDisableTiming));
        HIPCHK(h->events.make(&h->ev_join, hipEventDisableTiming));
        h->overlap_all = h->tun.overlap > 0;
    }
    TRY(make_plans(h));
    if (h->tun.place_trials > 1 && h->own_z && h->own_y && h->grid_slabs == 1)
        TRY(place_grids(h, (size_t)(G.nxl + G.hl + G.nhalo) * G.Ny * G.Nz, (size_t)G.nxl * G.Ny * G.Nzp));

    TRY(dmalloc(h, &h->V, (size_t)(M_MAX + 1) * n));
    if (h->n_slabs == 1 && !h->loc.on && h->tun.vq > 0) TRY(dmalloc(h, (char **)&h->vq, (size_t)16 * n));
    TRY(dmalloc(h, &h->pv_rows, pair_virial_rows((int)n)));
    TRY(dmalloc(h, &h->scal, (size_t)LZ_NSCAL));
    TRY(dmalloc(h, &h->lz_state, 1));
    HIPCHK(hipMemset(h->lz_state, 0, sizeof(LzState)));
    HIPCHK(h->pinned.make((void **)&h->sc_host, LZ_NSCAL * sizeof(double), hipHostMallocMapped));
    HIPCHK(hipHostGetDevicePointer((void **)&h->sc_host_dev, h->sc_host, 0));
    memset(h->sc_host, 0, LZ_NSCAL * sizeof(double));
    HIPCHK(h->events.make(&h->ev_scal, hipEventDisableTiming));
    if (!h->partials) {
        h->npart_cap = std::max(LZ_NPART, mreal_partials_needed((int)n + 1024));
        TRY(dmalloc(h, &h->partials, (size_t)LZ_NGRAM * h->npart_cap));
    }
    TRY(dmalloc(h, &h->lz_sums, (size_t)2 * LZ_NPART));
    for (auto &ph : h->ph) { HIPCHK(h->events.make(&ph.a)); HIPCHK(h->events.make(&ph.b)); }
    TRY(set_lanczos_op(h, h->tun.lz_op));
    h->info.device_bytes = h->bytes;
    if (h->tun.verbose) {
        fprintf(stderr, "--- NUFFT Hydrodynamics Statistics ---\nMx: %d\nMy: %d\nMz: %d\nrcut: %.6g\n"
                "Points per radius (x,y,z): %.4g, %.4g, %.4g\n--- Gaussian Spreading Parameters ---\ngauss_m: %.4g\ngauss_P: %d\n"
                "gauss_eta: %.6g\ngauss_w: %.6g\ngauss_gridh (x,y,z): %.6g, %.6g, %.6g\n"
                "--- engine ---\ncells: %d x %d x %d, ranks: %d (far-field slabs %d), device memory: %.2f GB\n",
                d.Nx, d.Ny, d.Nz, d.rcut, d.Nx / h->box.Lx, d.Ny / h->box.Ly, d.Nz / h->box.Lz, d.gaussm, d.P, d.eta,
                d.P * d.hx / 2.0, d.hx, d.hy, d.hz, h->nc.nx, h->nc.ny, h->nc.nz, h->n_slabs, h->grid_slabs, h->bytes / 1e9);
        fprintf(stderr, "grids at: real %p, spectra %p\n", (void *)h->rgrid, (void *)h->cgrid);
    }
    return 0;
}

extern "C" int pse_create(const pse_params *p, pse_handle **out) {
    if (!p || !out) return fail(PSE_ERR_INVALID, "null argument");
    *out = nullptr;
    pse_handle *h = new pse_handle();
    int r = create_impl(p, h);
    if (r) { std::string keep = error_text(); pse_destroy(h); error_text() = keep; return r; }
    *out = h;
    return 0;
}

extern "C" int pse_set_box(pse_handle *h, double Lx, double Ly, double Lz, double xy) {
    if (!h) return fail(PSE_ERR_INVALID, "null handle");
    if (!(Lx > 0 && Ly > 0 && Lz > 0)) return fail(PSE_ERR_INVALID, "box lengths must be positive");
    if (!(std::fabs(xy) <= 0.5 * (1.0 + 1e-9)))
        return fail(PSE_ERR_INVALID, "tilt xy = %g outside [-0.5, 0.5]: HOOMD flips the box there, and the sequential minimum image "
                    "(PSEv1/Mobility.cu:648) is exact only up to that tilt", xy);
    const Box nb{Lx, Ly, Lz, xy};
    const double gamma = std::max(std::fabs(xy), h->par.max_strain);
    DCells nc, nc_narrow;
    TRY(cells_for(nb, near_radius(h), gamma, h->n_slabs, h->tun.cell_bz, nc, h->loc.on ? 1 : 0));
    TRY(cells_for(nb, h->d.rcut, gamma, h->n_slabs, h->tun.cell_bz, nc_narrow, h->loc.on ? 1 : 0));
    if (h->loc.on && nc.nx != h->nc.nx)
        return fail(PSE_ERR_INVALID, "an owned-particle rank cannot change its cell layers along x (%d -> %d): the slabs are the ownership", h->nc.nx, nc.nx);
    if ((size_t)std::max(cells_total(nc), cells_total(nc_narrow)) > h->n_cells_alloc)
        return fail(PSE_ERR_INVALID, "box grew beyond the cell-list capacity sized at creation");
    TRY(gaussian_fits(h->d, Lx / h->d.Nx, Ly / h->d.Ny, Lz / h->d.Nz));
    h->box = nb;
    h->nc = nc;
    h->cell_gamma = gamma;
    h->nc_wide = h->skin_max > 0.0;
    h->d.hx = Lx / h->d.Nx; h->d.hy = Ly / h->d.Ny; h->d.hz = Lz / h->d.Nz;
    h->G.hx = h->d.hx; h->G.hy = h->d.hy; h->G.hz = h->d.hz;
    set_dbox(h);
    h->info.ncell_x = h->nc.nx; h->info.ncell_y = h->nc.ny; h->info.ncell_z = h->nc.nz;
    h->info.hx = h->d.hx; h->info.hy = h->d.hy; h->info.hz = h->d.hz;
    return 0;
}

extern "C" int pse_set_neighbor_skin(pse_handle *h, double r_buff) {
    if (!h) return fail(PSE_ERR_INVALID, "null handle");
    if (!(r_buff >= 0.0)) return fail(PSE_ERR_INVALID, "r_buff must be >= 0");
    if (r_buff > h->skin_max * (1 + 1e-12))
        return fail(PSE_ERR_INVALID, "r_buff = %g exceeds %g, what the cell grid and the list capacity were sized for at creation "
                    "(0 here: the neighbour list is not kept on this handle -- slab rank, cutoff too large for the box or the table)",
                    r_buff, h->skin_max);
    h->skin = r_buff;
    h->vl_valid = false;
    for (int q = 0; q < 2; ++q) { h->vl_misses[q] = 0; h->vl_suspend_left[q] = 0; h->vl_suspend_len[q] = 32; }
    return 0;
}
extern "C" int pse_neighbor_stats(pse_handle *h, double *r_buff, unsigned long long *builds, unsigned long long *reuses) {
    if (!h) return fail(PSE_ERR_INVALID, "null handle");
    if (r_buff) *r_buff = h->skin;
    if (builds) *builds = h->nlist_builds;
// ... 71 lines not shown
```

pse_amd/csrc/pse_handle.h:

```cpp
#pragma once
#include <hip/hip_runtime.h>
#include <rocfft/rocfft.h>

#include <type_traits>
#include <vector>

#include "../../include/pse_amd.h"
#include "pse_err.h"
#include "pse_host.h"
#include "pse_kernels.h"
#include "pse_farfield.h"
#include "pse_fft.h"
#include "pse_vectors.h"
#include "pse_local.h"

using namespace pse;

#define HIPCHK(x)                                                                                      \
    do {                                                                                               \
        hipError_t e_ = (x);                                                                           \
        if (e_ != hipSuccess) return fail(PSE_ERR_HIP, "%s failed: %s (%s:%d)", #x, hipGetErrorString(e_), __FILE__, __LINE__); \
    } while (0)
#define TRY(x)              \
    do {                    \
// ... 59 lines not shown
    ~Streams() { for (hipStream_t s : v) (void)hipStreamDestroy(s); }
    hipError_t make(hipStream_t *s, unsigned flags, const int *priority = nullptr) {
        *s = nullptr;
        const hipError_t e = priority ? hipStreamCreateWithPriority(s, flags, *priority) : hipStreamCreateWithFlags(s, flags);
        if (e == hipSuccess) v.push_back(*s);
        return e;
    }
    void synchronize() { for (hipStream_t s : v) (void)hipStreamSynchronize(s); }
private:
    std::vector<hipStream_t> v;
};
struct FftPlans {
    FftPlans() = default;
    FftPlans(const FftPlans &) = delete;
    ~FftPlans() { release(); }
    rocfft_status plan(rocfft_plan *p, rocfft_result_placement placement, rocfft_transform_type type, size_t dims, const size_t *len, size_t batch,
                       rocfft_plan_description desc) {
        *p = nullptr;
        const rocfft_status s = rocfft_plan_create(p, placement, type, rocfft_precision_double, dims, len, batch, desc);
        if (s == rocfft_status_success) plans.push_back(*p);
        return s;
    }
    rocfft_status info(rocfft_execution_info *i) {
        *i = nullptr;
        const rocfft_status s = rocfft_execution_info_create(i);
        if (s == rocfft_status_success) infos.push_back(*i);
        return s;
    }
    void release() {
        for (rocfft_plan p : plans) rocfft_plan_destroy(p);
        for (rocfft_execution_info i : infos) rocfft_execution_info_destroy(i);
        plans.clear(); infos.clear();
    }
private:
    std::vector<rocfft_plan> plans;
    std::vector<rocfft_execution_info> infos;
};

constexpr int PH_COUNT_ = 13;

struct Phase {
    hipEvent_t a = nullptr, b = nullptr;
};
struct DeviceObject;

struct pse_handle {
    pse_params par;
    Derived d;
    Box box;
    DBox dbox;
    DGrid G;
    DCells nc;
    double cell_gamma;
    int device = 0;
    hipStream_t stream = nullptr;
    hipStream_t wstream = nullptr;
    hipStream_t side = nullptr;
    hipStream_t side_owned = nullptr;
    int *bounds_host = nullptr;
    hipEvent_t ev_bounds = nullptr;
    bool bounds_pending = false;
    struct Tuning {
        int cell_bz = 6;
        double skin = 0.4;
        int overlap = 1;
        bool no_xfuse = false;
        int own_y_pow2 = 1;
        int own_y = 1;
        int own_z = 1;
        int yslab_regs = 1;
        int yfft_kb = 4;
        int wave_mode = 0;
        int spread_tz = 0, spread_nw = 0;
        int gather_bz = 0;
        int xmix_runtime = 0;
        int xfft_small_wide = 0;
        bool verbose = false;
        bool team_sstep = true;
        int team_sched[3] = {1, 2, 3};
        int vq = 1;
        int place_trials = 10;
        int lz_extra = 2;
        int lz_op = PSE_LANCZOS_RECORDS16;
    } tun;
    DCells bidx_nc = {0, 0, 0};
    hipEvent_t ev_fork = nullptr, ev_join = nullptr;
    bool overlap_all = false;
    bool side_on = false;
    hipEvent_t ev_scal = nullptr;
    int n_max = 0, n_pad = 0;
    unsigned *keys = nullptr, *keys_s = nullptr, *vals = nullptr, *perm = nullptr, *tag_s = nullptr;
    void *sort_tmp = nullptr;
    int *cell_cnt = nullptr;
    size_t sort_tmp_bytes = 0;
    int *cell_off = nullptr;
    double *pv_rows = nullptr;
    std::vector<DeviceObject *> topologies;
    DeviceArrays arrays;
    FftPlans fft;
    PinnedBuffers pinned;
    Streams streams;
    Events events;
    int *cnt_block = nullptr;
    size_t cnt_bins = 0;
    SpreadWork sw = {};
    NbList nb = {};
    double4 *nb64 = nullptr;
    int lz_op = PSE_LANCZOS_RECORDS16;
    bool nb_valid = false;
    bool lz_last_queued = false;
    double skin = 0.0;
    double skin_max = 0.0;
    VerletList vl = {};
    double4 *pos_build = nullptr;
    int *flags_host = nullptr;
    bool vl_valid = false;
    bool vl_use = false;
    bool vl_pending = false;
    int vl_N = 0; const unsigned *vl_group = nullptr; Box vl_box = {};
    bool nc_wide = false;
    unsigned long long nlist_builds = 0, nlist_reuses = 0;
    int vl_reused_since_build = 0, vl_misses[2] = {0, 0}, vl_suspend_left[2] = {0, 0}, vl_suspend_len[2] = {32, 32};
    int vl_kind = 0;
    bool pv_is_f = false;
    bool w_is_mpsi = false;
    bool sums0_done = false;
    CombineSink sink = {};
    bool tail_done = false;
    bool async_mode = false;
    bool gated = false;
    int *gate_word = nullptr;
    size_t n_cells_alloc = 0;
    float4 *posf_s = nullptr;
    double2 *pv = nullptr;
    double4 *pos_s = nullptr, *f_s = nullptr, *uw_s = nullptr, *ur_s = nullptr, *ub_s = nullptr, *psi_s = nullptr, *w_s = nullptr;
    double *coef = nullptr;
    int n_intervals = 0;
    double *rgrid = nullptr;
    double2 *cgrid = nullptr;
    rocfft_plan plan_fwd = nullptr, plan_inv = nullptr;
    rocfft_plan plan_x_fwd = nullptr, plan_x_inv = nullptr;
    rocfft_execution_info info_fwd = nullptr, info_inv = nullptr;
    int n_slabs = 1, slab_rank = 0, nyl = 0, y0 = 0;
    double2 *sendbuf = nullptr, *recvbuf = nullptr;
    int *d_bidx = nullptr, *d_bounds = nullptr;
    std::vector<int> row_lo, first_end, last_begin;
    std::vector<int> first2_end, last2_begin;
    double4 *w2_s = nullptr, *u_s = nullptr;
    double *sums_all = nullptr;
    double4 *utot_s = nullptr;
    bool xfuse = false;
    bool own_y = false;
    bool own_y_slab = false;
    int lz_extra = -1;
    void *vq = nullptr;
    int place_tried = 0; float place_ms_first = 0, place_ms_kept = 0;
    bool own_z = false;
    double2 *twiddle_z = nullptr;
    double2 *twiddle_y = nullptr;
    int grid_slabs = 1;
    double2 *twiddle = nullptr;
    void *fft_work = nullptr;
    size_t fft_work_bytes = 0;
    double4 *V = nullptr;
    double *scal = nullptr, *partials = nullptr;
    double *lz_sums = nullptr;
    double *sc_host = nullptr;
    double *sc_host_dev = nullptr;
    int *bounds_host_dev = nullptr;
    int npart_cap = 0;
    struct LocalPlan {
        bool on = false;
        LocalGeom g{};
        int rows_cap = 0;
        double *send[2] = {nullptr, nullptr}, *recv[2] = {nullptr, nullptr};
        size_t msg = 0;
        double4 *stage_w1 = nullptr, *stage_w2 = nullptr;
        double4 *porig_s = nullptr; double *mass_s = nullptr; int3 *image_s = nullptr;
        LocalRows *rows = nullptr;
        int *counters = nullptr;
        int *layer_cnt = nullptr;
        size_t zero_ints = 0;
        bool zeroed = false;
        int *err = nullptr, *err_host = nullptr;
        double *rd_send = nullptr, *rd_recv = nullptr;
        int *rd_rows = nullptr, *rd_off = nullptr, *rd_host = nullptr;
    } loc;
    LzState *lz_state = nullptr;
    unsigned long long lz_seq = 0;
    const uint32_t *ts_off = nullptr;
    pse_info info;
    bool timing = false;
    Phase ph[PH_COUNT_];
    unsigned long long bytes = 0;
    int sorted_N = 0;
    bool matvec_timed = false;
};

template <class T>
int dmalloc(pse_handle *h, T **p, size_t n) {
    if (n == 0) n = 1;
    const hipError_t e = h->arrays.make((void **)p, n * sizeof(T));
    if (e != hipSuccess) return fail(PSE_ERR_HIP, "hipMalloc((void **)p, n * sizeof(T)) failed: %s (%s:%d)", hipGetErrorString(e), __FILE__, __LINE__);
    h->bytes += n * sizeof(T);
    return 0;
}
int cells_for(const Box &box, double rc, double gamma, int n_slabs, int bz_want, DCells &out, int xpad = 0);
int bind_wave_stream(pse_handle *h);
ScaleArgs scale_args(pse_handle *h, bool noise, double kT, double dt, unsigned timestep, double xi = 0.0, double eta = 0.0);
bool team_sstep(const pse_handle *h);
void roctx_lookup();
struct PrepExtra { bool psi; unsigned timestep; };
int prepare(pse_handle *h, const double4 *pos, const double4 *vec, const unsigned *group, int N, bool defer_bounds, bool need_cells, PrepExtra px,
            bool with_real);


struct DeviceObject {
    pse_handle *h = nullptr;
    hipError_t err = hipSuccess;
    size_t bytes = 0;
    bool zeroed = false;
    DeviceObject() = default;
    virtual ~DeviceObject() = default;
    template <class T>
    hipError_t put(T **dst, const std::remove_const_t<T> *src, size_t n, bool zero = false) {
        *dst = nullptr;
        if (err != hipSuccess) return err;
        void *p = nullptr;
        bytes += n * sizeof(T);
        if ((err = arrays.make(&p, n * sizeof(T))) != hipSuccess) return err;
        *dst = (T *)p;
        if (src) err = hipMemcpy(p, src, n * sizeof(T), hipMemcpyHostToDevice);
        else if (zero) { err = hipMemset(p, 0, n * sizeof(T)); zeroed = true; }
        return err;
    }
private:
    DeviceArrays arrays;
};
```

pse_amd/csrc/pse_kernels.h:

```cpp
#pragma once
#include <hip/hip_runtime.h>
#include <stdint.h>

#include "pse_device.h"

namespace pse {

size_t cell_sort_temp_bytes(size_t ncell);
struct CellRanges {
    int n, c0[3], c1[3];
    __device__ __forceinline__ bool cell(int c) const {
        if (n == 0) return true;
        for (int q = 0; q < n; ++q) if (c >= c0[q] && c < c1[q]) return true;
        return false;
    }
    __device__ __forceinline__ bool row(int s, const int *__restrict__ cell_off) const {
        if (n == 0) return true;
        for (int q = 0; q < n; ++q) if (s >= cell_off[c0[q]] && s < cell_off[c1[q]]) return true;
        return false;
    }
};
struct RowMap {
    int n, lo[3], hi[3], base[3];
    __host__ __device__ int list_rows() const { return n ? base[n - 1] + ((hi[n - 1] - lo[n - 1] + 255) & ~255) : 0; }
// ... 27 lines not shown
    __device__ __forceinline__ RowMapRegs(const RowMap &m, const RowMap *dev) {
        n = m.n; l0 = m.lo[0]; l1 = m.lo[1]; l2 = m.lo[2]; h0 = m.hi[0]; h1 = m.hi[1]; h2 = m.hi[2]; b1 = m.base[1]; b2 = m.base[2];
        if (dev) { n = dev->n; l0 = dev->lo[0]; l1 = dev->lo[1]; l2 = dev->lo[2]; h0 = dev->hi[0]; h1 = dev->hi[1]; h2 = dev->hi[2]; b1 = dev->base[1]; b2 = dev->base[2]; }
    }
    __device__ __forceinline__ int list_rows() const { return n == 0 ? 0 : (n == 1 ? ((h0 - l0 + 255) & ~255) : (n == 2 ? b1 + ((h1 - l1 + 255) & ~255) : b2 + ((h2 - l2 + 255) & ~255))); }
    __device__ __forceinline__ int first_row() const { return h0 > l0 ? l0 : (n > 1 && h1 > l1 ? l1 : l2); }
    __device__ __forceinline__ int row(int lr) const {
        int l = l0, h = h0, b = 0;
        if (n > 1 && lr >= b1) { l = l1; h = h1; b = b1; }
        if (n > 2 && lr >= b2) { l = l2; h = h2; b = b2; }
        const int i = l + (lr - b);
        return i < h ? i : -1;
    }
};
inline RowMap row_map(int lo, int hi) { return RowMap{1, {lo, 0, 0}, {hi, 0, 0}, {0, 0, 0}}; }
inline RowMap row_map(const int (*rg)[2], int n) {
    RowMap m{};
    m.n = n;
    int base = 0;
    for (int k = 0; k < n; ++k) { m.lo[k] = rg[k][0]; m.hi[k] = rg[k][1]; m.base[k] = base; base += (rg[k][1] - rg[k][0] + 255) & ~255; }
    return m;
}

struct Gate {
    const int *word;
    int want;
    __device__ __forceinline__ bool closed() const { return word != nullptr && ((*word != 0) != (want != 0)); }
};
void launch_gate_decide(int *flags, int *word, hipStream_t s);
void launch_gate_zero(Gate g, int *a, size_t na, int *b, size_t nb, hipStream_t s);
void launch_gate_copy(Gate g, double4 *dst, const double4 *src, size_t n, hipStream_t s);
struct SlabBook { int n, cells_per_slab, spread, book[64]; };
hipError_t cell_sort(const double4 *pos, const unsigned *group, int N, DBox box, DCells nc, unsigned *keys, unsigned *rank,
                     unsigned *slots, int *cnt, int ncell, void *tmp, size_t tmp_bytes, int *cell_off, unsigned *perm, hipStream_t s,
                     CellRanges need = CellRanges{}, SlabBook sb = SlabBook{}, bool cnt_is_zero = false,
                     Gate gate = Gate{});
hipError_t launch_cell_scan(const int *cnt, int *out, int n, void *tmp, size_t tmp_bytes, hipStream_t s);
void launch_permute(const double4 *pos, const double4 *vec, const unsigned *group, const unsigned *perm, int N, DBox box,
                    double4 *pos_s, float4 *posf_s, double2 *pv, double4 *vec_s, unsigned *tag_s, hipStream_t s,
                    const double4 *pos_build = nullptr, double half_skin2 = 0.0, int *flags = nullptr,
                    CellRanges need = CellRanges{}, const int *cell_off = nullptr,
                    const struct FarBinArgs *far = nullptr,
                    double4 *psi_s = nullptr, uint32_t seed = 0, uint32_t timestep = 0,
                    Gate gate = Gate{}, const uint32_t *ts_off = nullptr);
void launch_permute_vec(const double4 *vec, const unsigned *tag_s, int N, double4 *vec_s, hipStream_t s);

struct NbList {
    char *data;
    int *cnt;
    int cap;
    double4 *c64;
};
__host__ __device__ inline size_t nb_list64_bytes(size_t rows, int cap) { return ((rows + 63) / 64) * (size_t)cap * 64 * 32; }
struct VerletList {
    unsigned *idx;
    int *cnt;
    int cap;
    int *flags;
    double rskin;
};
__host__ __device__ inline size_t verlet_list_bytes(size_t rows, int cap) { return ((rows + 63) / 64) * (size_t)(cap / 4) * 1024; }
enum { VL_NONE = 0, VL_WRITE = 1, VL_USE = 2 };
constexpr size_t NB_REC = 64 * 16;
__host__ __device__ inline size_t nb_list_bytes(size_t rows, int cap) { return ((rows + 63) / 64) * (size_t)cap * NB_REC; }
enum { MREAL_CELLS = 0, MREAL_BUILD_LIST = 1, MREAL_USE_LIST = 2 };
struct LzFuse {
    const double4 *vprev;
    double *partials;
    int npart_cap;
    const double4 *q, *p, *u;
    const double *upd;
    int n_upd;
};
enum { LZG_QW1 = 0, LZG_W1W1, LZG_W1W2, LZG_W2W2, LZG_PW1, LZG_PW2, LZG_UW2, LZG_QQ, LZ_NGRAM };
void launch_mreal(const double4 *pos_s, const float4 *posf_s, const double4 *vec_s, double4 *out_s, RowMap rows,
                  const int *cell_off, DBox box, DCells nc, double rcut, double self, const double *coef, int ncoef, NbList nb,
                  int mode, hipStream_t s, const double4 *vec2_s = nullptr, double4 *out2_s = nullptr,
                  VerletList vl = VerletList{}, int vl_mode = VL_NONE,
                  const double2 *pv = nullptr,
                  double *sums0 = nullptr, int sums0_cap = 0, double *scal = nullptr,
                  Gate gate = Gate{},
                  DevRowArgs dr = DevRowArgs{});
bool mreal_table_in_lds(int ncoef);
void launch_mreal_lanczos(const double4 *pos_s, const double4 *vec_s, double4 *w, RowMap rows, const int *cell_off,
                          DBox box, DCells nc, double rcut, double self, const double *coef, NbList nb, LzFuse lz,
                          double *scal, hipEvent_t ev_begin, hipEvent_t ev_end, hipStream_t s,
                          VerletList vl = VerletList{},
                          int sums = 1,
                          const int *stop = nullptr,
                          DevRowArgs dr = DevRowArgs{},
                          const void *vec_q = nullptr,
                          bool no_reduce = false);
int mreal_partials_needed(int rows);
void launch_eval_fg(const double *r, int n, const double *coef, double *f, double *g, hipStream_t s);

}
```

pse_amd/csrc/pse_kernels.hip:

```cpp
#include "pse_kernels.h"
#include "pse_vectors.h"
#include "pse_farbin.h"

#include <hipcub/hipcub.hpp>

namespace pse {

constexpr unsigned KEY_FOREIGN = 0xFFFFFFFFu;
__global__ void k_cell_keys(const double4 *__restrict__ pos, const unsigned *__restrict__ group, int N, DBox box,
                            DCells nc, unsigned *__restrict__ keys, unsigned *__restrict__ rank, int *__restrict__ cnt, CellRanges need,
                            SlabBook sb, Gate gate) {
    if (gate.closed()) return;
    const int g = blockIdx.x * blockDim.x + threadIdx.x;
    const bool live = g < N;
    unsigned key = 0;
    bool mine = false;
    if (live) {
        const unsigned idx = group ? group[g] : (unsigned)g;
        const double4 p = pos[idx];
        double fx, fy, fz;
        frac_coords(box, p.x, p.y, p.z, fx, fy, fz);
        const int cx = cell_coord(fx, nc.nx), cy = cell_coord(fy, nc.ny), cz = cell_coord(fz, nc.nz);
        const int zb = cz / nc.bz;
        key = (unsigned)cell_slot(nc, cx, cy, zb, cz - zb * nc.bz);
// ... 500 lines not shown
        unsigned e[U] = {e4.x, e4.y, e4.z, e4.w};
        double2 a[U], b[U], c[U];
        double4 G[U];
#pragma unroll
        for (int u = 0; u < U; ++u) {
            if (u && s0 + u >= cnt) e[u] = e[0];
            if (PK) {
                const double2 *r = pv + 3 * (size_t)e[u];
                a[u] = r[0]; b[u] = r[1]; c[u] = r[2];
            } else {
                const double4 pj = pos_s[e[u]], Fj = vec_s[e[u]];
                a[u] = make_double2(pj.x, pj.y); b[u] = make_double2(pj.z, Fj.x); c[u] = make_double2(Fj.y, Fj.z);
            }
            if (TWO) G[u] = vec2_s[e[u]];
        }
#pragma unroll
        for (int u = 0; u < U; ++u) {
            double dx = pi.x - a[u].x, dy = pi.y - a[u].y, dz = pi.z - b[u].x;
            const double ny = rint(dy * box.iLy);
            dy -= ny * box.Ly; dx -= ny * box.xy * box.Ly;
            const double nx = rint(dx * box.iLx), nz = rint(dz * box.iLz);
            dx -= nx * box.Lx; dz -= nz * box.Lz;
            const double r2 = dx * dx + dy * dy + dz * dz;
            const bool in = s0 + u < cnt && r2 < rcut2 && r2 > 0.0;
            double f, h;
            eval_fg<2 * RS_NCOEF + 1>(fmin(r2, rcut2), scoef, f, h);
            if (!in) { f = 0.0; h = 0.0; }
            const double Fx = b[u].y, Fy = c[u].x, Fz = c[u].y;
            if (!LIST || TWO) {
                const double rd = (dx * Fx + dy * Fy + dz * Fz) * h;
                ux += f * Fx + rd * dx; uy += f * Fy + rd * dy; uz += f * Fz + rd * dz;
            }
            if (LIST && F64) {
                const PairCoef64 pc = pair_coef64(f, h, dx, dy, dz);
                if (TWO) pair_apply64(pc, G[u].x, G[u].y, G[u].z, wx, wy, wz);
                else pair_apply64(pc, Fx, Fy, Fz, ux, uy, uz);
                if (in) {
                    if (total < nb.cap) nb_store64(rec, rec64, total, lane, e[u], pc);
                    ++total;
                }
            } else if (LIST) {
                const PairCoef pc = pair_coef(f, h, dx, dy, dz);
                if (TWO) pair_apply(pc, G[u].x, G[u].y, G[u].z, wx, wy, wz);
                else pair_apply(pc, Fx, Fy, Fz, ux, uy, uz);
                if (in) {
                    if (total < nb.cap) nb_store(rec, total, lane, e[u], pc);
                    ++total;
                }
            } else if (TWO) {
                const double sd = (dx * G[u].x + dy * G[u].y + dz * G[u].z) * h;
                wx += f * G[u].x + sd * dx; wy += f * G[u].y + sd * dy; wz += f * G[u].z + sd * dz;
            }
        }
    }
    out_s[i] = make_double4(ux, uy, uz, 0.0);
    if (TWO) out2_s[i] = make_double4(wx, wy, wz, 0.0);
    if (LIST) nb.cnt[i] = total > nb.cap ? -1 : total;
}

__device__ __forceinline__ void eval_fg_lean(double r2, const double *__restrict__ coef, double &f, double &gmf_r2) {
    const double ir = rsqrt(r2), r = r2 * ir, ir2 = ir * ir;
    double f0, g0;
    if (r > 2.0) { const double ir3 = ir * ir2; f0 = 0.75 * ir + 0.5 * ir3; g0 = 1.5 * ir - ir3; }
    else { f0 = 1.0 - 0.28125 * r; g0 = 1.0 - 0.1875 * r; }
    const double s = r * RS_PER_UNIT;
    const int k = (int)s;
    const double t = 2.0 * (s - k) - 1.0;
    const double *c = coef + (size_t)k * (2 * RS_NCOEF);
    double fw = c[RS_DEG], gw = c[RS_NCOEF + RS_DEG];
#pragma unroll 1
    for (int q = RS_DEG - 1; q >= 0; --q) {
        fw = fma(fw, t, c[q]);
        gw = fma(gw, t, c[RS_NCOEF + q]);
    }
    f = f0 - fw;
    gmf_r2 = ((g0 - gw) - f) * ir2;
}

template <int FUSE, int UNROLL, int NT, int WSP = 1, bool VQ = false, bool F64 = false>
__global__ void __launch_bounds__(NT, (WSP == 4 ? 5 : 1))
k_mreal_list(const double4 *__restrict__ pos_s, const double4 *__restrict__ vec_s, double4 *__restrict__ out_s, RowMap rm_arg,
             DBox box, double self, NbList nb, LzFuse lz,
             const int *__restrict__ cell_off, DCells nc, double rcut2, const double *__restrict__ coef, VerletList vl,
             const int *__restrict__ stop, DevRowArgs dr, const vq4 *__restrict__ vec_q = nullptr) {
    if (stop && *stop) return;
    const RowMapRegs rm(rm_arg, dr.rm);
    int nb_live = gridDim.x;
    if (dr.rm) {
        nb_live = (rm.list_rows() + (WSP > 1 ? 64 : NT) - 1) / (WSP > 1 ? 64 : NT);
        if ((int)blockIdx.x >= nb_live) {
            if (FUSE && threadIdx.x == 0)
                for (int t = 0; t < (FUSE == 2 || FUSE == 3 ? (int)LZ_NGRAM : 3); ++t) lz.partials[(size_t)t * lz.npart_cap + blockIdx.x] = 0.0;
            return;
        }
    }
    __shared__ double sh[4];
    static_assert(WSP == 1 || NT == 64 * WSP, "split rows: one wave per slot phase");
    const int wv = WSP > 1 ? (int)(threadIdx.x >> 6) : 0;
    const int lr = WSP > 1 ? xcd_block(blockIdx.x, nb_live) * 64 + (int)(threadIdx.x & 63)
                           : xcd_block(blockIdx.x, nb_live) * NT + (int)threadIdx.x;
    const int i = rm.row(lr);
    const bool active = i >= 0;
    double ux = 0.0, uy = 0.0, uz = 0.0;
    double4 vi = make_double4(0.0, 0.0, 0.0, 0.0);
    if (active) {
        vi = vec_s[i];
        const int cnt = nb.cnt[i];
        if (cnt >= 0) {
            if (wv == 0) { ux = self * vi.x; uy = self * vi.y; uz = self * vi.z; }
            const int lane = lr & 63;
            const char *rec = nb.data + (size_t)(lr >> 6) * nb.cap * NB_REC;
            static_assert(UNROLL == 4, "one list group per iteration");
            for (int s0 = UNROLL * wv; s0 < cnt; s0 += UNROLL * WSP) {
                const char *grp = rec + (size_t)(s0 >> 2) * (4 * NB_REC);
                unsigned e[UNROLL];
                nb4 c[UNROLL];
                d4v c64[F64 ? UNROLL : 1];
#pragma unroll
                for (int u = 0; u < UNROLL; ++u) {
                    c[u] = __builtin_nontemporal_load((const nb4 *)grp + u * 64 + lane);
                    if (F64) c64[u] = __builtin_nontemporal_load((const d4v *)nb.c64 + (size_t)(lr >> 6) * nb.cap * 64 + (size_t)(s0 >> 2) * 256 + u * 64 + lane);
                    e[u] = c[u].x;
                    if (u && s0 + u >= cnt) e[u] = e[0];
                }
                double2 vxy[UNROLL];
                double vz[UNROLL];
                vq4 vq[UNROLL];
#pragma unroll
                for (int u = 0; u < UNROLL; ++u) {
                    if (VQ && !F64) { vq[u] = vec_q[e[u] & JMASK]; continue; }
                    const double4 *vj = vec_s + (e[u] & JMASK);
                    vxy[u] = *reinterpret_cast<const double2 *>(vj);
                    vz[u] = vj->z;
                }
#pragma unroll
                for (int u = 0; u < UNROLL; ++u) {
                    const bool ok = s0 + u < cnt;
                    if (F64) {
                        const PairCoef64 pc{ok ? c64[u].x : 0.0, ok ? c64[u].y : 0.0, ok ? c64[u].z : 0.0, ok ? c64[u].w : 0.0, (c[u].x & NB_NEG) != 0u};
                        pair_apply64(pc, vxy[u].x, vxy[u].y, vz[u], ux, uy, uz);
                        continue;
                    }
                    const PairCoef pc = nb_unpack(c[u], ok);
                    if (VQ) { vq_unpack(vq[u], vxy[u].x, vxy[u].y, vz[u]); }
                    pair_apply(pc, vxy[u].x, vxy[u].y, vz[u], ux, uy, uz);
                }
            }
        } else if (wv != 0) {
        } else if (vl.idx) {
            const double4 pi = pos_s[i];
            ux = self * vi.x; uy = self * vi.y; uz = self * vi.z;
            const int lane = i & 63, vc = vl.cnt[i];
            const char *vrec = (const char *)vl.idx + (size_t)(i >> 6) * (vl.cap / 4) * 1024;
            for (int sl = 0; sl < vc; ++sl) {
                const unsigned j = ((const unsigned *)(vrec + (size_t)(sl >> 2) * 1024))[lane * 4 + (sl & 3)];
                const double4 pj = pos_s[j];
                double dx = pi.x - pj.x, dy = pi.y - pj.y, dz = pi.z - pj.z;
                min_image(box, dx, dy, dz);
                const double r2 = dx * dx + dy * dy + dz * dz;
                if (r2 < rcut2 && r2 > 0.0) {
                    double f, h;
                    eval_fg_lean(r2, coef, f, h);
                    const double4 Fj = vec_s[j];
                    if (F64) pair_apply64(pair_coef64(f, h, dx, dy, dz), Fj.x, Fj.y, Fj.z, ux, uy, uz);
                    else pair_apply(pair_coef(f, h, dx, dy, dz), Fj.x, Fj.y, Fj.z, ux, uy, uz);
                }
            }
        } else {
            const double4 pi = pos_s[i];
            ux = self * vi.x; uy = self * vi.y; uz = self * vi.z;
            double fx, fy, fz;
            frac_coords(box, pi.x, pi.y, pi.z, fx, fy, fz);
            const int cx = cell_coord(fx, nc.nx), cy = cell_coord(fy, nc.ny), cz = cell_coord(fz, nc.nz);
            for_each_run(nc, cell_off, cx, cy, cz, [&](int jb, int je, unsigned) {
                for (int j = jb; j < je; ++j) {
                    const double4 pj = pos_s[j];
                    double dx = pi.x - pj.x, dy = pi.y - pj.y, dz = pi.z - pj.z;
                    min_image(box, dx, dy, dz);
                    const double r2 = dx * dx + dy * dy + dz * dz;
                    if (r2 < rcut2 && j != i && r2 > 0.0) {
                        double f, h;
                        eval_fg_lean(r2, coef, f, h);
                        const double4 Fj = vec_s[j];
                        if (F64) pair_apply64(pair_coef64(f, h, dx, dy, dz), Fj.x, Fj.y, Fj.z, ux, uy, uz);
                        else pair_apply(pair_coef(f, h, dx, dy, dz), Fj.x, Fj.y, Fj.z, ux, uy, uz);
                    }
                }
            });
        }
    }
    if (WSP > 1) {
        __shared__ double red[WSP > 1 ? (WSP - 1) * 3 * 64 : 1];
        const int ln = threadIdx.x & 63;
        if (wv > 0) { red[((wv - 1) * 3 + 0) * 64 + ln] = ux; red[((wv - 1) * 3 + 1) * 64 + ln] = uy; red[((wv - 1) * 3 + 2) * 64 + ln] = uz; }
        __syncthreads();
        if (wv > 0) return;
        for (int w = 0; w < WSP - 1; ++w) { ux += red[(w * 3 + 0) * 64 + ln]; uy += red[(w * 3 + 1) * 64 + ln]; uz += red[(w * 3 + 2) * 64 + ln]; }
    }
    if (FUSE == 2 || FUSE == 3) {
        double g[LZ_NGRAM];
#pragma unroll
        for (int t = 0; t < LZ_NGRAM; ++t) g[t] = 0.0;
        if (active) {
            auto dot = [](const double4 &x, double yx, double yy, double yz) { return x.x * yx + x.y * yy + x.z * yz; };
            const double4 z4 = make_double4(0.0, 0.0, 0.0, 0.0);
            const double4 p = lz.p ? lz.p[i] : z4;
            if (FUSE == 2) {
                const double4 q = lz.q[i], u = lz.u ? lz.u[i] : z4;
                g[LZG_QW1] = dot(q, vi.x, vi.y, vi.z); g[LZG_W1W1] = dot(vi, vi.x, vi.y, vi.z); g[LZG_W1W2] = dot(vi, ux, uy, uz);
                g[LZG_W2W2] = ux * ux + uy * uy + uz * uz; g[LZG_PW1] = dot(p, vi.x, vi.y, vi.z);
                g[LZG_PW2] = dot(p, ux, uy, uz); g[LZG_UW2] = dot(u, ux, uy, uz); g[LZG_QQ] = dot(q, q.x, q.y, q.z);
            } else {
                g[LZG_QW1] = dot(vi, ux, uy, uz); g[LZG_W1W1] = ux * ux + uy * uy + uz * uz; g[LZG_PW1] = dot(p, ux, uy, uz);
                g[LZG_QQ] = dot(vi, vi.x, vi.y, vi.z);
            }
        }
        static_assert(FUSE < 2 || FUSE == 4 || NT == 64 || WSP > 1, "Gram sums: one wave per block of rows");
#pragma unroll
        for (int t = 0; t < LZ_NGRAM; ++t) {
            if (FUSE == 3 && t != LZG_QW1 && t != LZG_W1W1 && t != LZG_PW1 && t != LZG_QQ) { if (threadIdx.x == 0) lz.partials[(size_t)t * lz.npart_cap + blockIdx.x] = 0.0; continue; }
            const double v = wave_sum(g[t]);
            if (threadIdx.x == 0) lz.partials[(size_t)t * lz.npart_cap + blockIdx.x] = v;
        }
    } else if (FUSE == 4) {
        static_assert(FUSE != 4 || NT == 64 || WSP > 1, "one wave per block of rows");
        const double b = wave_sum(active ? vi.x * ux + vi.y * uy + vi.z * uz : 0.0);
        if (threadIdx.x == 0) lz.partials[lz.npart_cap + blockIdx.x] = b;
    } else if (FUSE) {
        double a = 0.0, b = 0.0, c = 0.0;
        if (active) {
            a = vi.x * vi.x + vi.y * vi.y + vi.z * vi.z;
            b = vi.x * ux + vi.y * uy + vi.z * uz;
            if (lz.vprev) {
                const double4 m = lz.vprev[i];
                c = vi.x * m.x + vi.y * m.y + vi.z * m.z;
            }
        }
        if (NT == 64 || WSP > 1) { a = wave_sum(a); b = wave_sum(b); c = wave_sum(c); }
        else { a = block_sum(a, sh); __syncthreads(); b = block_sum(b, sh); __syncthreads(); c = block_sum(c, sh); }
        if (threadIdx.x == 0) {
            lz.partials[blockIdx.x] = a; lz.partials[lz.npart_cap + blockIdx.x] = b; lz.partials[2 * lz.npart_cap + blockIdx.x] = c;
        }
    }
    if (active) {
        out_s[i] = make_double4(ux, uy, uz, 0.0);
        if (dr.stage_hi) {
            const int lb = dr.lr->last_begin, no = dr.lr->n_own;
            if (i >= lb && i < no && i - lb < dr.stage_cap) dr.stage_hi[i - lb] = make_double4(ux, uy, uz, 0.0);
        }
    }
}

static size_t mreal_lds_bytes(int ncoef) { return (size_t)(ncoef / (2 * RS_NCOEF)) * (2 * RS_NCOEF + 1) * sizeof(double); }
bool mreal_table_in_lds(int ncoef) { return mreal_lds_bytes(ncoef) <= 14 * 1024; }

void launch_mreal(const double4 *pos_s, const float4 *posf_s, const double4 *vec_s, double4 *out_s, RowMap rm,
                  const int *cell_off, DBox box, DCells nc, double rcut, double self, const double *coef, int ncoef, NbList nb,
                  int mode, hipStream_t s, const double4 *vec2_s, double4 *out2_s, VerletList vl, int vl_mode, const double2 *pv,
                  double *sums0, int sums0_cap, double *scal, Gate gate, DevRowArgs dr) {
    const int rows = dr.rm ? dr.rows_cap : rm.list_rows();
    if (rows <= 0) return;
    const dim3 g(nblocks(rows, TPB)), b(TPB);
    const size_t cb = mreal_lds_bytes(ncoef);
    const bool cl = mreal_table_in_lds(ncoef);
    const bool f64 = nb.c64 != nullptr;
    if (mode == MREAL_USE_LIST) {
        if (f64) hipLaunchKernelGGL((k_mreal_list<0, 4, TPB, 1, false, true>), g, b, 0, s, pos_s, vec_s, out_s, rm, box, self, nb, LzFuse{}, cell_off, nc, rcut * rcut, coef,
                                    vl_mode == VL_USE ? vl : VerletList{}, nullptr, DevRowArgs{}, nullptr);
        else hipLaunchKernelGGL((k_mreal_list<0, 4, TPB>), g, b, 0, s, pos_s, vec_s, out_s, rm, box, self, nb, LzFuse{}, cell_off, nc, rcut * rcut, coef,
                                vl_mode == VL_USE ? vl : VerletList{}, nullptr, DevRowArgs{});
        return;
    }
    const bool list = mode == MREAL_BUILD_LIST, two = list && vec2_s != nullptr;
    if (vl_mode == VL_USE) {
        const int hi = rm.hi[0];
#define PSE_VERLET(L, T, F) do { if (pv) hipLaunchKernelGGL((k_mreal_verlet<L, T, true, F>), g, b, cb, s, pos_s, pv, vec_s, out_s, hi, box, rcut * rcut, self, coef, ncoef, nb, vl, two ? vec2_s : nullptr, out2_s, gate); \
        else hipLaunchKernelGGL((k_mreal_verlet<L, T, false, F>), g, b, cb, s, pos_s, pv, vec_s, out_s, hi, box, rcut * rcut, self, coef, ncoef, nb, vl, two ? vec2_s : nullptr, out2_s, gate); } while (0)
        if (list && two) { if (f64) PSE_VERLET(true, true, true); else PSE_VERLET(true, true, false); }
        else if (list) { if (f64) PSE_VERLET(true, false, true); else PSE_VERLET(true, false, false); }
        else PSE_VERLET(false, false, false);
#undef PSE_VERLET
        return;
    }
    const bool wr = vl_mode == VL_WRITE && cl;
    const double cmax = 1.5 * (box.Lx + std::fabs(box.xy) * box.Ly + box.Ly + box.Lz);
    const double rpre = (wr ? vl.rskin : rcut) + 16.0 * cmax * 5.97e-8;
    const float rcut2_pre = (float)(rpre * rpre * (1.0 + 1e-6));
#define PSE_CELLS_F(L, C, T, V, F) hipLaunchKernelGGL((k_mreal_cells<L, C, T, V, false, false, F>), g, b, (C) ? cb : 0, s, pos_s, posf_s, vec_s, out_s, rm, cell_off, box, nc, rcut * rcut, rcut2_pre, self, coef, ncoef, nb, two ? vec2_s : nullptr, out2_s, vl, (two && (C)) ? sums0 : nullptr, sums0_cap, gate, dr, nullptr)
#define PSE_CELLS_PK_F(L, T, D, F) hipLaunchKernelGGL((k_mreal_cells<L, true, T, false, D, true, F>), g, b, cb, s, pos_s, posf_s, vec_s, out_s, rm, cell_off, box, nc, rcut * rcut, rcut2_pre, self, coef, ncoef, nb, two ? vec2_s : nullptr, out2_s, vl, (two && !(D)) ? sums0 : nullptr, sums0_cap, gate, dr, pv)
#define PSE_CELLS(L, C, T, V) do { if ((L) && f64) PSE_CELLS_F(L, C, T, V, (L)); else PSE_CELLS_F(L, C, T, V, false); } while (0)
#define PSE_CELLS_PK(L, T, D) do { if ((L) && f64) PSE_CELLS_PK_F(L, T, D, (L)); else PSE_CELLS_PK_F(L, T, D, false); } while (0)
    if (dr.rm) {
        if (list && two) PSE_CELLS_PK(true, true, true); else PSE_CELLS_PK(false, false, true);
        return;
    }
    if (pv && cl && !wr && vl_mode != VL_USE && (two || !list)) {
        if (list) PSE_CELLS_PK(true, true, false); else PSE_CELLS_PK(false, false, false);
    } else if (list) {
        if (cl && two) { if (wr) PSE_CELLS(true, true, true, true); else PSE_CELLS(true, true, true, false); }
        else if (cl) { if (wr) PSE_CELLS(true, true, false, true); else PSE_CELLS(true, true, false, false); }
        else PSE_CELLS(true, false, false, false);
    } else if (cl) { if (wr) PSE_CELLS(false, true, false, true); else PSE_CELLS(false, true, false, false); }
    else PSE_CELLS(false, false, false, false);
#undef PSE_CELLS_PK
#undef PSE_CELLS
#undef PSE_CELLS_PK_F
#undef PSE_CELLS_F
    if (sums0 && list && two && cl)
        launch_lz_reduce(sums0, (int)g.x * (TPB / 64), sums0_cap, 3, scal, nullptr, s);
}

int mreal_partials_needed(int rows) { return nblocks(std::max(rows, 1), 64); }
void launch_mreal_lanczos(const double4 *pos_s, const double4 *vec_s, double4 *w, RowMap rm, const int *cell_off,
                          DBox box, DCells nc, double rcut, double self, const double *coef, NbList nb, LzFuse lz,
                          double *scal, hipEvent_t ev_begin, hipEvent_t ev_end, hipStream_t s, VerletList vl,
                          int sums, const int *stop, DevRowArgs dr, const void *vec_q, bool no_reduce) {
    const int rows = std::max(dr.rm ? dr.rows_cap : rm.list_rows(), 1);
    if (ev_begin) (void)hipEventRecord(ev_begin, s);
    const int nb64 = nblocks(rows, 64);
#define PSE_LIST(F) hipLaunchKernelGGL((k_mreal_list<F, 4, 256, 4>), dim3(nb64), dim3(256), 0, s, pos_s, vec_s, w, rm, box, self, nb, lz, cell_off, nc, rcut * rcut, coef, vl, stop, dr)
#define PSE_LIST64(F) hipLaunchKernelGGL((k_mreal_list<F, 4, 256, 4, false, true>), dim3(nb64), dim3(256), 0, s, pos_s, vec_s, w, rm, box, self, nb, lz, cell_off, nc, rcut * rcut, coef, vl, stop, dr, nullptr)
    if (nb.c64) {
        if (sums == 0) PSE_LIST64(0); else if (sums == 1) PSE_LIST64(1); else if (sums == 2) PSE_LIST64(2); else if (sums == 3) PSE_LIST64(3); else PSE_LIST64(4);
    } else if (sums == 1 && vec_q)
        hipLaunchKernelGGL((k_mreal_list<1, 4, 256, 4, true>), dim3(nb64), dim3(256), 0, s, pos_s, vec_s, w, rm, box, self, nb, lz, cell_off, nc, rcut * rcut, coef, vl, stop, dr,
                           (const vq4 *)vec_q);
    else if (sums == 4 && vec_q)
        hipLaunchKernelGGL((k_mreal_list<4, 4, 256, 4, true>), dim3(nb64), dim3(256), 0, s, pos_s, vec_s, w, rm, box, self, nb, lz, cell_off, nc, rcut * rcut, coef, vl, stop, dr,
                           (const vq4 *)vec_q);
    else if (sums == 0) PSE_LIST(0); else if (sums == 1) PSE_LIST(1); else if (sums == 2) PSE_LIST(2); else if (sums == 3) PSE_LIST(3); else PSE_LIST(4);
#undef PSE_LIST64
#undef PSE_LIST
    if (ev_end) (void)hipEventRecord(ev_end, s);
    if (no_reduce) return;
    if (sums == 4) launch_lz_reduce_split(lz.partials + lz.npart_cap, nb64, lz.upd, lz.n_upd, scal, stop, s);
    else if (sums >= 1) launch_lz_reduce(lz.partials, nb64, lz.npart_cap, sums == 1 ? 3 : (int)LZ_NGRAM, scal, stop, s);
}

__global__ void k_eval_fg(const double *__restrict__ r, int n, const double *__restrict__ coef, double *f, double *g) {
    const int i = blockIdx.x * blockDim.x + threadIdx.x;
    if (i >= n) return;
    double ff, h;
    const double r2 = r[i] * r[i];
    eval_fg(r2, coef, ff, h);
    f[i] = ff;
    g[i] = ff + h * r2;
}
void launch_eval_fg(const double *r, int n, const double *coef, double *f, double *g, hipStream_t s) {
    hipLaunchKernelGGL(k_eval_fg, dim3(nblocks(n, TPB)), dim3(TPB), 0, s, r, n, coef, f, g);
}

}
```

pse_amd/csrc/pse_vectors.h:

```cpp
#pragma once
#include "pse_host.h"
#include "pse_kernels.h"

namespace pse {

void launch_psi(double4 *psi_s, const unsigned *tag_s, int N, uint32_t seed, uint32_t timestep, hipStream_t s,
                CellRanges need = CellRanges{}, const int *cell_off = nullptr);
constexpr int LZ_TMP = 257, LZ_UU = 272, LZ_NSCAL = 400;
constexpr int LZ_NPART = 1024;
void launch_lz_reduce(const double *partials, int npart, int cap, int nsum, double *scal, const int *stop, hipStream_t s);
struct BasisCoef { double t[104]; };
struct CombineSink { bool on; const double4 *add_a, *add_b; const unsigned *tag_s; double4 *vel; double4 *rows; };
void launch_basis_combine(const double4 *x0, const double4 *V, size_t stride, const BasisCoef &t, int m, const double *scal,
                          double scale, int use_norm, double4 *out_s, int lo, int hi, hipStream_t s, CombineSink sink = CombineSink{},
                          const struct LzState *st = nullptr);
void launch_lz_dots(const double4 *x, const double4 *y, const double4 *vprev, int lo, int hi, double *partials, int cap,
                    double *scal, hipStream_t s);
struct LzBlockArgs {
    const double4 *q, *p, *w1, *w2;
    double4 *u;
    double4 *v1, *v2;
    int j;
};
void launch_lz_block(const LzBlockArgs &a, bool full, double *scal, const int (*row_ranges)[2], int n_ranges, hipStream_t s,
                     const double *sums_all = nullptr, int nranks = 0, double *sch = nullptr,
                     const RowRanges *rg_dev = nullptr, int rows_cap = 0,
                     bool vectors_off = false, const int *stop = nullptr);
void launch_vq_roundtrip(const double *in, double *out, int n, hipStream_t s);
int lz_update_grid(int rows);
void launch_lz_reduce_split(const double *xy, int n_xy, const double *upd, int n_upd, double *scal, const int *stop, hipStream_t s);
void launch_lz_update(const double4 *xin, const double4 *y, const double4 *xprev, double4 *xnext, int j,
                      double *scal, const int (*row_ranges)[2], int n_ranges, hipStream_t s,
                      const double *sums_all = nullptr, int nranks = 0, double *sch = nullptr, const int *stop = nullptr,
                      void *xq = nullptr,
                      double *next_sums = nullptr);
constexpr int LZ_HOST_M = 380, LZ_HOST_STEPNORM = 381, LZ_HOST_STATUS = 382, LZ_HOST_SEQ = 383, LZ_HOST_OPEN = 384;
void launch_lz_decide(const LzDecide &d, double *scal, LzState *st, double *sch, double seq, hipStream_t s);
bool lz_decide_supported(int m_hi);
void launch_sum_rows(const double4 *a, const double4 *b, const double4 *c, double4 *out, int lo, int hi, hipStream_t s,
                     const unsigned *tag_s = nullptr);
void launch_pick(const int *cell_off, const int *idx, int n, int *out, hipStream_t s);
void launch_scatter_sum(const double4 *a, const double4 *b, const double4 *c, const unsigned *tag_s, int N,
                        double4 *vel, hipStream_t s);
void launch_integrate(double4 *pos, const double4 *vel, double3 *accel, int3 *image, const double4 *force,
                      const unsigned *group, int N, DBox box, double dt, double shear_rate, hipStream_t s);
void launch_add_inplace(double *a, const double *b, size_t n, hipStream_t s);
struct CopyList { int n; const double *src[40]; double *dst[40]; unsigned cnt[40]; };
void launch_copy_list(const CopyList &l, hipStream_t s);

}
```

pse_amd/csrc/pse_vectors.hip:

```cpp
#include "pse_vectors.h"

namespace pse {

__global__ void k_psi(double4 *__restrict__ psi_s, const unsigned *__restrict__ tag_s, int N, uint32_t seed,
                      uint32_t timestep, CellRanges need, const int *__restrict__ cell_off) {
    const int s = blockIdx.x * blockDim.x + threadIdx.x;
    if (s >= N || !need.row(s, cell_off)) return;
    uint32_t r[4];
    philox4x32(tag_s[s], 0u, timestep, DOMAIN_PARTICLE, seed, PHILOX_KEY1, r);
    const double q = 1.7320508075688772;
    psi_s[s] = make_double4(uniform_pm(r[0], q), uniform_pm(r[1], q), uniform_pm(r[2], q), 0.0);
}
void launch_psi(double4 *psi_s, const unsigned *tag_s, int N, uint32_t seed, uint32_t timestep, hipStream_t s, CellRanges need,
                const int *cell_off) {
    hipLaunchKernelGGL(k_psi, dim3(nblocks(N, TPB)), dim3(TPB), 0, s, psi_s, tag_s, N, seed, timestep, need, cell_off);
}

static inline int vec_grid(int N) { return std::min(LZ_NPART, std::max(1, nblocks(N, TPB))); }

__global__ void __launch_bounds__(TPB)
k_lz_dots(const double4 *__restrict__ x, const double4 *__restrict__ y, const double4 *__restrict__ vprev, int lo, int hi,
          double *__restrict__ partials, int cap) {
    __shared__ double sh[4];
    double a = 0.0, b = 0.0, c = 0.0;
    for (int i = lo + blockIdx.x * TPB + threadIdx.x; i < hi; i += gridDim.x * TPB) {
        const double4 p = x[i];
        a += p.x * p.x + p.y * p.y + p.z * p.z;
        if (y) { const double4 q = y[i]; b += p.x * q.x + p.y * q.y + p.z * q.z; }
        if (vprev) { const double4 m = vprev[i]; c += p.x * m.x + p.y * m.y + p.z * m.z; }
    }
    a = block_sum(a, sh);
    __syncthreads();
    b = block_sum(b, sh);
    __syncthreads();
    c = block_sum(c, sh);
    if (threadIdx.x == 0) { partials[blockIdx.x] = a; partials[cap + blockIdx.x] = b; partials[2 * cap + blockIdx.x] = c; }
}
__global__ void __launch_bounds__(1024)
k_lz_reduce(const double *__restrict__ partials, int npart, int cap, int nsum, double *__restrict__ scal, const int *__restrict__ stop,
            const double *__restrict__ upd, int n_upd) {
    if (stop && *stop) return;
    __shared__ double sh[16];
    const int q = blockIdx.x;
    const double *p = partials + (size_t)q * cap;
    if (upd) { p = q == 1 ? partials : upd + (q == 2 ? LZ_NPART : 0); if (q != 1) npart = n_upd; }
    double v = 0.0;
    for (int i = threadIdx.x; i < npart; i += 1024) v += p[i];
    v = wave_sum(v);
    if ((threadIdx.x & 63) == 0) sh[threadIdx.x >> 6] = v;
    __syncthreads();
    if (threadIdx.x == 0) {
        double t = 0.0;
        for (int w = 0; w < 16; ++w) t += sh[w];
        scal[LZ_TMP + q] = t;
    }
}
void launch_lz_reduce(const double *partials, int npart, int cap, int nsum, double *scal, const int *stop, hipStream_t s) {
    hipLaunchKernelGGL(k_lz_reduce, dim3(nsum), dim3(1024), 0, s, partials, npart, cap, nsum, scal, stop, (const double *)nullptr, 0);
}
void launch_lz_reduce_split(const double *xy, int n_xy, const double *upd, int n_upd, double *scal, const int *stop, hipStream_t s) {
    hipLaunchKernelGGL(k_lz_reduce, dim3(3), dim3(1024), 0, s, xy, n_xy, 0, 3, scal, stop, upd, n_upd);
}
__global__ void __launch_bounds__(TPB)
k_lz_update(const double4 *__restrict__ xin, const double4 *__restrict__ y, const double4 *__restrict__ xprev,
            double4 *__restrict__ xnext, int j, double *__restrict__ scal, RowRanges rg,
            const double *__restrict__ sums_all, int nranks, double *__restrict__ sch, const int *__restrict__ stop, vq4 *__restrict__ xq,
            double *__restrict__ next_sums) {
    if (stop && *stop) return;
    double s1 = 0.0, s2 = 0.0, s3raw = 0.0;
    if (nranks > 0) for (int r = 0; r < nranks; ++r) { s1 += sums_all[r * LZ_NGRAM]; s2 += sums_all[r * LZ_NGRAM + 1]; s3raw += sums_all[r * LZ_NGRAM + 2]; }
    else { s1 = scal[LZ_TMP]; s2 = scal[LZ_TMP + 1]; s3raw = scal[LZ_TMP + 2]; }
    const double bprev = j == 1 ? scal[LZ_NORM] : (j > 1 ? scal[LZ_BETA + j - 1] : 0.0);
    const double ibprev = bprev > 0.0 ? 1.0 / bprev : 0.0;
    const double beta = s1 > 0.0 ? sqrt(s1) : 0.0;
    const double inv = beta > 0.0 ? 1.0 / beta : 0.0;
    const double alpha = s1 > 0.0 ? s2 / s1 - s3raw * ibprev : 0.0;
    if (blockIdx.x == 0 && threadIdx.x == 0) {
        scal[LZ_ALPHA + j] = alpha;
        if (j == 0) { scal[LZ_NORM] = beta; scal[LZ_BETA] = 0.0; } else scal[LZ_BETA + j] = beta;
        if (sch) {
            sch[LZ_ALPHA + j] = alpha;
            if (j == 0) { sch[LZ_NORM] = beta; sch[LZ_BETA] = 0.0; } else sch[LZ_BETA + j] = beta;
        }
    }
    const double cp = beta * ibprev;
    const int n0 = rg.hi[0] - rg.lo[0], n1 = rg.n > 1 ? rg.hi[1] - rg.lo[1] : 0, n2 = rg.n > 2 ? rg.hi[2] - rg.lo[2] : 0;
    double nn = 0.0, np = 0.0;
    for (int t = blockIdx.x * TPB + threadIdx.x; t < n0 + n1 + n2; t += gridDim.x * TPB) {
        const int i = t < n0 ? rg.lo[0] + t : (t < n0 + n1 ? rg.lo[1] + (t - n0) : rg.lo[2] + (t - n0 - n1));
        const double4 p = xin[i], q = y[i];
        double nx = (q.x - alpha * p.x) * inv, ny = (q.y - alpha * p.y) * inv, nz = (q.z - alpha * p.z) * inv;
        if (xprev) { const double4 m = xprev[i]; nx -= cp * m.x; ny -= cp * m.y; nz -= cp * m.z; }
        xnext[i] = make_double4(nx, ny, nz, 0.0);
        if (xq) xq[i] = vq_pack(nx, ny, nz);
        nn += nx * nx + ny * ny + nz * nz;
        np += nx * p.x + ny * p.y + nz * p.z;
    }
    if (next_sums) {
        __shared__ double sh[2][4];
        nn = wave_sum(nn); np = wave_sum(np);
        if ((threadIdx.x & 63) == 0) { sh[0][threadIdx.x >> 6] = nn; sh[1][threadIdx.x >> 6] = np; }
        __syncthreads();
        if (threadIdx.x == 0) {
            next_sums[blockIdx.x] = sh[0][0] + sh[0][1] + sh[0][2] + sh[0][3];
            next_sums[LZ_NPART + blockIdx.x] = sh[1][0] + sh[1][1] + sh[1][2] + sh[1][3];
        }
    }
}
template <bool FULL>
__global__ void __launch_bounds__(TPB)
k_lz_block(LzBlockArgs a, double *__restrict__ scal, RowRanges rg, const double *__restrict__ sums_all, int nranks, double *__restrict__ sch,
           const RowRanges *__restrict__ rg_dev, int vectors_off, const int *__restrict__ stop) {
    if (stop && *stop) return;
    if (rg_dev) { rg = *rg_dev; if (vectors_off) rg.n = 0; }
    __shared__ double sG[LZ_NGRAM];
    if (threadIdx.x < LZ_NGRAM) {
        double v = 0.0;
        for (int r = 0; r < nranks; ++r) v += sums_all[r * LZ_NGRAM + threadIdx.x];
        sG[threadIdx.x] = nranks > 0 ? v : scal[LZ_TMP + threadIdx.x];
    }
    __syncthreads();
    double G[LZ_NGRAM];
#pragma unroll
    for (int t = 0; t < LZ_NGRAM; ++t) G[t] = sG[t];
    const int j = a.j;
    const double n0 = G[LZG_QQ], s2 = n0 > 0.0 ? 1.0 / n0 : 0.0, sc = sqrt(s2);
    const double beta = j > 0 ? scal[LZ_BETA + j] : 0.0, alpha_prev = j > 0 ? scal[LZ_ALPHA + j - 1] : 0.0;
    const double ga = G[LZG_QW1] * s2, gb = G[LZG_W1W1] * s2, gf = G[LZG_PW1] * sc;
    const double alpha = ga;
    const double bp2 = gb - alpha * alpha - 2.0 * beta * gf + beta * beta;
    const double bp = bp2 > 0.0 ? sqrt(bp2) : 0.0, ibp = bp > 1e-12 ? 1.0 / bp : 0.0;
    double alpha1 = 0.0, bpp = 0.0, ibpp = 0.0, uu_next = 0.0;
    if (FULL) {
        const double gc = G[LZG_W1W2] * s2, gd = G[LZG_W2W2] * s2, ge = gb , gg = G[LZG_PW2] * sc, gg2 = gg ,
                     gh = G[LZG_UW2] * sc, gk = j > 0 ? scal[LZ_UU + j] : 0.0, gf2 = gf ;
        const double r1w2 = gc - alpha * ge - beta * gg, r1w1 = gb - alpha * ga - beta * gf, r1u = gg2 - alpha * gf2 - beta * alpha_prev;
        alpha1 = (r1w2 - alpha * r1w1 - beta * r1u) * ibp * ibp;
        const double zz = (gd + alpha * alpha * gb + beta * beta * gk - 2.0 * alpha * gc - 2.0 * beta * gh + 2.0 * alpha * beta * gg2) * ibp * ibp;
        const double qz = (ge - alpha * ga - beta * gf2) * ibp;
        const double bpp2 = zz - alpha1 * alpha1 - 2.0 * bp * qz + bp * bp;
        bpp = bpp2 > 0.0 ? sqrt(bpp2) : 0.0;
        ibpp = bpp > 1e-12 ? 1.0 / bpp : 0.0;
        uu_next = zz;
    } else {
        uu_next = gb;
    }
    if (blockIdx.x == 0 && threadIdx.x == 0) {
        if (j == 0) { scal[LZ_NORM] = n0 > 0.0 ? sqrt(n0) : 0.0; scal[LZ_BETA] = 0.0; }
        scal[LZ_ALPHA + j] = alpha;
        scal[LZ_BETA + j + 1] = bp;
        if (FULL) { scal[LZ_ALPHA + j + 1] = alpha1; scal[LZ_BETA + j + 2] = bpp; }
        scal[LZ_UU + j + (FULL ? 2 : 1)] = uu_next;
        if (sch) {
            if (j == 0) { sch[LZ_NORM] = n0 > 0.0 ? sqrt(n0) : 0.0; sch[LZ_BETA] = 0.0; }
            sch[LZ_ALPHA + j] = alpha;
            sch[LZ_BETA + j + 1] = bp;
            if (FULL) { sch[LZ_ALPHA + j + 1] = alpha1; sch[LZ_BETA + j + 2] = bpp; }
        }
    }
    const int n0r = rg.n > 0 ? rg.hi[0] - rg.lo[0] : 0, n1r = rg.n > 1 ? rg.hi[1] - rg.lo[1] : 0, n2r = rg.n > 2 ? rg.hi[2] - rg.lo[2] : 0;
    for (int t = blockIdx.x * TPB + threadIdx.x; t < n0r + n1r + n2r; t += gridDim.x * TPB) {
        const int i = t < n0r ? rg.lo[0] + t : (t < n0r + n1r ? rg.lo[1] + (t - n0r) : rg.lo[2] + (t - n0r - n1r));
        const double4 q = a.q[i], w1 = a.w1[i];
        double4 p = make_double4(0.0, 0.0, 0.0, 0.0), u = p;
        if (j > 0) { p = a.p[i]; if (FULL) u = a.u[i]; }
        const double qx = sc * q.x, qy = sc * q.y, qz_ = sc * q.z, ax = sc * w1.x, ay = sc * w1.y, az = sc * w1.z;
        const double v1x = (ax - alpha * qx - beta * p.x) * ibp, v1y = (ay - alpha * qy - beta * p.y) * ibp, v1z = (az - alpha * qz_ - beta * p.z) * ibp;
        a.v1[i] = make_double4(v1x, v1y, v1z, 0.0);
        double nx = v1x, ny = v1y, nz = v1z;
        if (FULL) {
            const double4 w2 = a.w2[i];
            const double z1x = (sc * w2.x - alpha * ax - beta * u.x) * ibp, z1y = (sc * w2.y - alpha * ay - beta * u.y) * ibp,
                         z1z = (sc * w2.z - alpha * az - beta * u.z) * ibp;
            nx = (z1x - alpha1 * v1x - bp * qx) * ibpp; ny = (z1y - alpha1 * v1y - bp * qy) * ibpp; nz = (z1z - alpha1 * v1z - bp * qz_) * ibpp;
            a.v2[i] = make_double4(nx, ny, nz, 0.0);
            a.u[i] = make_double4(z1x, z1y, z1z, 0.0);
// ... 97 lines not shown
    extern __shared__ double lds[];
    __shared__ double tbuf[2][104];
    __shared__ int okf[2];
    if (a.first) { if (threadIdx.x == 0) { st->done = 0; st->m_final = 0; st->checked = 0; st->status = 0; st->stepnorm = 1.0; } }
    else if (st->done) return;
    __syncthreads();
    const int wv = threadIdx.x >> 6, nm = a.m_hi - a.m_lo + 1;
    const double *alpha = scal + LZ_ALPHA, *beta = scal + LZ_BETA;
    const double norm = scal[LZ_NORM];
    const bool dead = !(norm > 0.0) || !isfinite(norm);
    if (wv < nm && !dead) {
        const int m = a.m_lo + wv;
        double *base = lds + (wv == 0 ? 0 : (size_t)a.m_lo * a.m_lo);
        const bool ok = lz_sqrt_e1(m, alpha, beta, base, tbuf[wv]);
        if ((threadIdx.x & 63) == 0) okf[wv] = ok ? 1 : 0;
    }
    __shared__ double s_alpha[104], s_beta[104], s_prev[104];
    __shared__ int s_checked;
    __shared__ double s_stepnorm;
    for (int q = threadIdx.x; q <= min(a.m_hi, 103); q += blockDim.x) { s_alpha[q] = scal[LZ_ALPHA + q]; s_beta[q] = scal[LZ_BETA + q]; s_prev[q] = st->t_prev[q]; }
    if (threadIdx.x == 0) { s_checked = a.first ? 0 : st->checked; s_stepnorm = a.first ? 1.0 : st->stepnorm; }
    __syncthreads();
    if (threadIdx.x != 0) return;
    alpha = s_alpha; beta = s_beta;
    int m_final = 0, status = 0, checked = s_checked;
    double stepnorm = s_stepnorm;
    const double *t_fin = nullptr;
    if (dead) { m_final = -1; }
    else if (a.pending_beta > 0 && beta[a.pending_beta] < 1e-8) {
        m_final = a.pending_beta; stepnorm = 0.0; t_fin = s_prev;
    } else {
        for (int w = 0; w < nm && !m_final; ++w) {
            const int m = a.m_lo + w;
            const bool have_beta = m < a.done_iters || a.have_last_beta;
            if (!isfinite(alpha[m - 1]) || (have_beta && !isfinite(beta[m])) || !okf[w]) { m_final = max(checked, 1); status = 2; t_fin = checked ? s_prev : tbuf[w]; break; }
            const double *tc = tbuf[w];
            if (m < a.done_iters && beta[m] < 1e-8) { m_final = m; stepnorm = 0.0; t_fin = tc; break; }
            if (checked == m - 1 && checked > 0) {
                double s2 = tc[m - 1] * tc[m - 1];
                for (int q = 0; q < m - 1; ++q) { const double dq = tc[q] - s_prev[q]; s2 += dq * dq; }
                stepnorm = sqrt(s2 / alpha[0]);
                if (stepnorm <= a.tol || m >= a.m_max) { m_final = m; t_fin = tc; break; }
            }
            if (a.have_last_beta && m == a.done_iters && beta[m] < 1e-8) { m_final = m; stepnorm = 0.0; t_fin = tc; break; }
            for (int q = 0; q < m; ++q) { st->t_prev[q] = tc[q]; s_prev[q] = tc[q]; }
            checked = m;
        }
        if (!m_final && (a.last || a.done_iters >= a.m_max)) {
            m_final = checked; t_fin = s_prev; status = a.done_iters >= a.m_max ? 0 : 1;
        }
    }
    st->checked = checked;
    st->stepnorm = stepnorm;
    if (m_final) {
        const int m = max(m_final, 0);
        for (int q = 0; q < m; ++q) st->coef[q] = t_fin[q] / (q == 0 ? norm : (a.normalised ? 1.0 : beta[q]));
        st->m_final = m; st->status = status;
        st->done = 1;
        if (sch) {
            sch[LZ_HOST_M] = (double)m; sch[LZ_HOST_STEPNORM] = stepnorm; sch[LZ_HOST_STATUS] = (double)status; sch[LZ_HOST_SEQ] = seq;
            if (status != 0) sch[LZ_HOST_OPEN] = sch[LZ_HOST_OPEN] + 1.0;
        }
    }
}
static size_t lz_decide_lds(int m_lo, int m_hi) {
    size_t n = (size_t)m_lo * m_lo;
    if (m_hi != m_lo) n += (size_t)m_hi * m_hi;
    return n * sizeof(double);
}
bool lz_decide_supported(int m_hi) { return m_hi >= 1 && m_hi <= 100 && lz_decide_lds(std::max(1, m_hi - 1), m_hi) <= 150 * 1024; }
void launch_lz_decide(const LzDecide &d, double *scal, LzState *st, double *sch, double seq, hipStream_t s) {
    const size_t lds = lz_decide_lds(d.m_lo, d.m_hi);
    static LdsAttr attr;
    if (lds > 48 * 1024 && attr.need(150 * 1024)) (void)hipFuncSetAttribute((const void *)k_lz_decide, hipFuncAttributeMaxDynamicSharedMemorySize, 150 * 1024);
    hipLaunchKernelGGL(k_lz_decide, dim3(1), dim3(128), lds, s, d, scal, st, sch, seq);
}

void launch_lz_dots(const double4 *x, const double4 *y, const double4 *vprev, int lo, int hi, double *partials, int cap,
                    double *scal, hipStream_t s) {
    const int g = vec_grid(std::max(1, hi - lo));
    hipLaunchKernelGGL(k_lz_dots, dim3(g), dim3(TPB), 0, s, x, y, vprev, lo, hi, partials, cap);
    launch_lz_reduce(partials, g, cap, y ? 3 : 1, scal, nullptr, s);
}
void launch_lz_update(const double4 *xin, const double4 *y, const double4 *xprev, double4 *xnext, int j,
                      double *scal, const int (*rg)[2], int nrg, hipStream_t s, const double *sums_all, int nranks, double *sch,
                      const int *stop, void *xq, double *next_sums) {
    RowRanges r{};
    r.n = nrg;
    int total = 0;
    for (int q = 0; q < nrg && q < 3; ++q) { r.lo[q] = rg[q][0]; r.hi[q] = rg[q][1]; total += rg[q][1] - rg[q][0]; }
    if (total <= 0) next_sums = nullptr;
    hipLaunchKernelGGL(k_lz_update, dim3(vec_grid(std::max(1, total))), dim3(TPB), 0, s, xin, y, xprev, xnext, j, scal, r, sums_all, nranks, sch, stop, (vq4 *)xq, next_sums);
}
int lz_update_grid(int rows) { return vec_grid(std::max(1, rows)); }
__global__ void k_vq_roundtrip(const double *__restrict__ in, double *__restrict__ out, int n) {
    const int i = blockIdx.x * blockDim.x + threadIdx.x;
    if (i >= n) return;
    double x, y, z;
    vq_unpack(vq_pack(in[3 * i], in[3 * i + 1], in[3 * i + 2]), x, y, z);
    out[3 * i] = x; out[3 * i + 1] = y; out[3 * i + 2] = z;
}
void launch_vq_roundtrip(const double *in, double *out, int n, hipStream_t s) {
    hipLaunchKernelGGL(k_vq_roundtrip, dim3(nblocks(n, TPB)), dim3(TPB), 0, s, in, out, n);
}
__global__ void k_sum_rows(const double4 *__restrict__ a, const double4 *__restrict__ b, const double4 *__restrict__ c,
                           double4 *__restrict__ out, int lo, int hi, const unsigned *__restrict__ tag_s) {
    const int i = lo + blockIdx.x * blockDim.x + threadIdx.x;
    if (i >= hi) return;
    double x = 0, y = 0, z = 0;
    if (a) { const double4 v = a[i]; x += v.x; y += v.y; z += v.z; }
    if (b) { const double4 v = b[i]; x += v.x; y += v.y; z += v.z; }
    if (c) { const double4 v = c[i]; x += v.x; y += v.y; z += v.z; }
    out[i] = make_double4(x, y, z, tag_s ? (double)tag_s[i] : 0.0);
}
void launch_sum_rows(const double4 *a, const double4 *b, const double4 *c, double4 *out, int lo, int hi, hipStream_t s,
                     const unsigned *tag_s) {
    if (hi > lo) hipLaunchKernelGGL(k_sum_rows, dim3(nblocks(hi - lo, TPB)), dim3(TPB), 0, s, a, b, c, out, lo, hi, tag_s);
}
__global__ void k_pick(const int *__restrict__ cell_off, const int *__restrict__ idx, int n, int *__restrict__ out) {
    const int r = blockIdx.x * blockDim.x + threadIdx.x;
    if (r < n) out[r] = cell_off[idx[r]];
}
void launch_pick(const int *cell_off, const int *idx, int n, int *out, hipStream_t s) {
    hipLaunchKernelGGL(k_pick, dim3(nblocks(n, TPB)), dim3(TPB), 0, s, cell_off, idx, n, out);
}

__global__ void __launch_bounds__(TPB)
k_basis_combine(const double4 *__restrict__ x0, const double4 *__restrict__ V, size_t stride, BasisCoef tc, int m,
                const double *__restrict__ scal, double scale, int use_norm, double4 *__restrict__ out, int lo, int N, CombineSink sink,
                const LzState *__restrict__ st) {
    const double *t = tc.t;
    if (st) { m = st->m_final; t = st->coef; }
    const double sc = use_norm ? scale * scal[LZ_NORM] : scale;
    for (int i = lo + blockIdx.x * TPB + threadIdx.x; i < N; i += gridDim.x * TPB) {
        double x = 0, y = 0, z = 0;
        for (int q = 0; q < m; ++q) {
            const double4 v = q == 0 ? x0[i] : V[(size_t)q * stride + i];
            const double tq = t[q];
            x += tq * v.x; y += tq * v.y; z += tq * v.z;
        }
        x *= sc; y *= sc; z *= sc;
        if (!sink.on) { out[i] = make_double4(x, y, z, 0.0); continue; }
        double sx = 0.0, sy = 0.0, sz = 0.0;
        if (sink.add_a) { const double4 v = sink.add_a[i]; sx += v.x; sy += v.y; sz += v.z; }
        if (sink.add_b) { const double4 v = sink.add_b[i]; sx += v.x; sy += v.y; sz += v.z; }
        sx += x; sy += y; sz += z;
        const unsigned idx = sink.tag_s[i];
        if (sink.vel) { double4 o = sink.vel[idx]; o.x = sx; o.y = sy; o.z = sz; sink.vel[idx] = o; }
        else sink.rows[i] = make_double4(sx, sy, sz, (double)idx);
    }
}
void launch_basis_combine(const double4 *x0, const double4 *V, size_t stride, const BasisCoef &t_dev, int m, const double *scal,
                          double scale, int use_norm, double4 *out_s, int lo, int hi, hipStream_t s, CombineSink sink, const LzState *st) {
    hipLaunchKernelGGL(k_basis_combine, dim3(std::min(2048, std::max(1, nblocks(hi - lo, TPB)))), dim3(TPB), 0, s, x0, V, stride,
                       t_dev, m, scal, scale, use_norm, out_s, lo, hi, sink, st);
}

__global__ void k_scatter_sum(const double4 *__restrict__ a, const double4 *__restrict__ b,
                              const double4 *__restrict__ c, const unsigned *__restrict__ tag_s, int N,
                              double4 *__restrict__ vel) {
    const int s = blockIdx.x * blockDim.x + threadIdx.x;
    if (s >= N) return;
    double x = 0, y = 0, z = 0;
    if (a) { const double4 v = a[s]; x += v.x; y += v.y; z += v.z; }
    if (b) { const double4 v = b[s]; x += v.x; y += v.y; z += v.z; }
    if (c) { const double4 v = c[s]; x += v.x; y += v.y; z += v.z; }
    const unsigned idx = tag_s ? tag_s[s] : (unsigned)a[s].w;
    double4 o = vel[idx];
    o.x = x; o.y = y; o.z = z;
    vel[idx] = o;
}
void launch_scatter_sum(const double4 *a, const double4 *b, const double4 *c, const unsigned *tag_s, int N,
                        double4 *vel, hipStream_t s) {
    hipLaunchKernelGGL(k_scatter_sum, dim3(nblocks(N, TPB)), dim3(TPB), 0, s, a, b, c, tag_s, N, vel);
}

__global__ void k_integrate(double4 *__restrict__ pos, const double4 *__restrict__ vel, double3 *__restrict__ accel,
                            int3 *__restrict__ image, const double4 *__restrict__ force,
                            const unsigned *__restrict__ group, int N, DBox box, double dt, double shear_rate) {
    const int g = blockIdx.x * blockDim.x + threadIdx.x;
    if (g >= N) return;
    const unsigned idx = group ? group[g] : (unsigned)g;
    double4 p = pos[idx];
    const double4 v = vel[idx];
    const double4 F = force[idx];
    p.x += (v.x + shear_rate * p.y) * dt;
    p.y += v.y * dt;
    p.z += v.z * dt;
    int3 im = image[idx];
    double n = floor(p.z * box.iLz + 0.5);
    p.z -= n * box.Lz; im.z += (int)n;
    n = floor(p.y * box.iLy + 0.5);
    p.y -= n * box.Ly; p.x -= n * box.xy * box.Ly; im.y += (int)n;
    n = floor((p.x - box.xy * p.y) * box.iLx + 0.5);
    p.x -= n * box.Lx; im.x += (int)n;
    const double im_ = 1.0 / v.w;
    accel[idx] = make_double3(F.x * im_, F.y * im_, F.z * im_);
    pos[idx] = p;
    image[idx] = im;
}
void launch_integrate(double4 *pos, const double4 *vel, double3 *accel, int3 *image, const double4 *force,
                      const unsigned *group, int N, DBox box, double dt, double shear_rate, hipStream_t s) {
    hipLaunchKernelGGL(k_integrate, dim3(nblocks(N, TPB)), dim3(TPB), 0, s, pos, vel, accel, image, force, group, N,
                       box, dt, shear_rate);
}
__global__ void k_axpy_inplace(double *__restrict__ a, const double *__restrict__ b, size_t n) {
    for (size_t i = (size_t)blockIdx.x * blockDim.x + threadIdx.x; i < n; i += (size_t)gridDim.x * blockDim.x) a[i] += b[i];
}
__global__ void __launch_bounds__(TPB) k_copy_list(CopyList l) {
    const int it = blockIdx.y;
    const double *__restrict__ src = l.src[it];
    double *__restrict__ dst = l.dst[it];
    const unsigned n = l.cnt[it];
    if ((((size_t)src | (size_t)dst) & 15) == 0) {
        const unsigned n2 = n >> 1;
        for (unsigned i = blockIdx.x * TPB + threadIdx.x; i < n2; i += gridDim.x * TPB) ((double2 *)dst)[i] = ((const double2 *)src)[i];
        if ((n & 1) && blockIdx.x == 0 && threadIdx.x == 0) dst[n - 1] = src[n - 1];
    } else {
        for (unsigned i = blockIdx.x * TPB + threadIdx.x; i < n; i += gridDim.x * TPB) dst[i] = src[i];
    }
}
void launch_copy_list(const CopyList &l, hipStream_t s) {
    if (l.n <= 0) return;
    unsigned mx = 0;
    for (int i = 0; i < l.n; ++i) mx = std::max(mx, l.cnt[i]);
    const int gx = std::max(1, std::min(256, nblocks((long)(mx / 2 + 1), TPB)));
    hipLaunchKernelGGL(k_copy_list, dim3(gx, l.n), dim3(TPB), 0, s, l);
}
void launch_add_inplace(double *a, const double *b, size_t n, hipStream_t s) {
    hipLaunchKernelGGL(k_axpy_inplace, dim3(std::min<long>(2048, nblocks((long)n, TPB))), dim3(TPB), 0, s, a, b, n);
}

}
```

Measured before the change: 334.4 million particle-steps/s.

## Store Lanczos basis vectors in packed 24-byte rows instead of double4

```diff
diff --git a/pse_amd/csrc/pse_capi.hip b/pse_amd/csrc/pse_capi.hip
--- a/pse_amd/csrc/pse_capi.hip
+++ b/pse_amd/csrc/pse_capi.hip
@@ -743,11 +743,25 @@
 
 static int update_ranges(const pse_handle *h, int N, int rg[3][2]) { return row_ranges(h, N, 1, rg); }
 
-static double4 *lz_vec(const pse_handle *h, int q) { return q < 0 ? nullptr : q == 0 ? h->psi_s : h->V + (size_t)q * h->n_pad; }
+static VecOut lz_vec(const pse_handle *h, int q) {
+    if (q < 0) return VecOut(nullptr);
+    if (q == 0) return VecOut(h->psi_s);
+    if (h->rows24) return VecOut(reinterpret_cast<double *>(h->V) + (size_t)3 * q * h->n_pad, 1);
+    return VecOut(h->V + (size_t)q * h->n_pad);
+}
+static double4 *lz_vec4(const pse_handle *h, int q) { return reinterpret_cast<double4 *>(lz_vec(h, q).p); }
+static VecIn lz_basis(const pse_handle *h) { return VecIn(reinterpret_cast<const double *>(h->V), h->rows24 ? 1 : 0); }
+static VecOut lz_y(const pse_handle *h, bool from_list) { return from_list && h->rows24 ? VecOut(h->w24, 1) : VecOut(h->w_s); }
+static int lz_real_ok(const pse_handle *h, int j) {
+    if (j > 0 && h->rows24)
+        return fail(PSE_ERR_INVALID, "Lanczos iteration %d would walk the cells on a basis in 24-byte rows: the pair list of this call is "
+                    "no longer valid (was the Lanczos operator changed after the list was built?); repeat the call", j);
+    return 0;
+}
 static LzBlockArgs lz_block_args(const pse_handle *h, int j, bool full) {
     LzBlockArgs a{};
-    a.q = lz_vec(h, j); a.p = lz_vec(h, j - 1); a.w1 = h->w_s; a.w2 = full ? h->w2_s : nullptr;
-    a.u = h->u_s; a.v1 = lz_vec(h, j + 1); a.v2 = full ? lz_vec(h, j + 2) : nullptr;
+    a.q = lz_vec4(h, j); a.p = lz_vec4(h, j - 1); a.w1 = h->w_s; a.w2 = full ? h->w2_s : nullptr;
+    a.u = h->u_s; a.v1 = lz_vec4(h, j + 1); a.v2 = full ? lz_vec4(h, j + 2) : nullptr;
     a.j = j;
     return a;
 }
@@ -788,7 +802,7 @@
     for (pse_handle *h : act(T)) {
         int lo, hi;
         row_range(h, N, lo, hi);
-        launch_basis_combine(h->psi_s, h->V, h->n_pad, tc, st.m_final, h->scal, scale, 1, h->ub_s, lo, hi, h->stream, h->sink);
+        launch_basis_combine(h->psi_s, lz_basis(h), h->n_pad, tc, st.m_final, h->scal, scale, 1, h->ub_s, lo, hi, h->stream, h->sink);
         h->tail_done = h->sink.on;
         h->info.lanczos_m = st.m_final; h->info.lanczos_matvecs = matvecs; h->info.lanczos_stepnorm = st.stepnorm;
         h->info.lanczos_exchanges = exchanges;
@@ -804,8 +818,9 @@
     h->lz_last_queued = true;
     int rg[3][2];
     const int nrg_all = update_ranges(h, N, rg);
+    VecOut y = lz_y(h, false);
     auto vector_part = [&](int j, const int *gate) {
-        launch_lz_update(lz_vec(h, j), h->w_s, lz_vec(h, j - 1), lz_vec(h, j + 1), j, h->scal, rg, nrg_all, h->stream,
+        launch_lz_update(lz_vec(h, j), y, lz_vec(h, j - 1), lz_vec(h, j + 1), j, h->scal, rg, nrg_all, h->stream,
                          nullptr, 0, h->sc_host_dev, gate, vq_of(h), h->lz_sums);
     };
     auto iteration = [&](int j, bool scalars_only, const int *gate) -> int {
@@ -813,18 +828,20 @@
         const bool fused = !have_y && h->nb.cap > 0 && h->nb_valid;
         if (!fused && !have_y) {
             if (gate) return fail(PSE_ERR_NUMERIC, "queued Lanczos: a gated iteration needs the pair list");
+            TRY(lz_real_ok(h, j));
             TRY(real(T, j == 0 ? &pse_handle::psi_s : &pse_handle::V, &pse_handle::w_s, (size_t)j * h->n_pad, 0, N, true));
         }
-        const double4 *vjm1 = lz_vec(h, j - 1);
+        y = lz_y(h, fused);
+        const double4 *vjm1 = lz_vec4(h, j - 1);
         const bool split = fused && j > 0;
         if (fused)
-            launch_mreal_lanczos(h->pos_s, lz_vec(h, j), h->w_s, row_map(0, N), h->cell_off, h->dbox, h->nc, h->d.rcut, h->d.self, h->coef, h->nb,
+            launch_mreal_lanczos(h->pos_s, lz_vec(h, j), y, row_map(0, N), h->cell_off, h->dbox, h->nc, h->d.rcut, h->d.self, h->coef, h->nb,
                                  LzFuse{split ? nullptr : vjm1, h->partials, h->npart_cap, nullptr, nullptr, nullptr, h->lz_sums, lz_update_grid(N)}, h->scal, nullptr, nullptr, h->stream,
                                  h->vl_use ? h->vl : VerletList{}, split ? 4 : 1, gate, DevRowArgs{}, j > 0 ? vq_of(h) : nullptr);
         else if (!(j == 0 && h->sums0_done))
-            launch_lz_dots(lz_vec(h, j), h->w_s, vjm1, 0, N, h->partials, h->npart_cap, h->scal, h->stream);
+            launch_lz_dots(lz_vec4(h, j), h->w_s, vjm1, 0, N, h->partials, h->npart_cap, h->scal, h->stream);
         h->w_is_mpsi = false; h->sums0_done = false;
-        if (scalars_only) launch_lz_update(lz_vec(h, j), h->w_s, vjm1, lz_vec(h, j + 1), j, h->scal, rg, 0, h->stream, nullptr, 0,
+        if (scalars_only) launch_lz_update(lz_vec(h, j), y, lz_vec(h, j - 1), lz_vec(h, j + 1), j, h->scal, rg, 0, h->stream, nullptr, 0,
                                            h->sc_host_dev, gate);
         else vector_part(j, gate);
         return 0;
@@ -844,7 +861,7 @@
     TRY(te(h, PH_LANCZOS));
     if (before_first_wait) TRY(before_first_wait());
     if (before_combine) TRY(before_combine());
-    launch_basis_combine(h->psi_s, h->V, h->n_pad, BasisCoef{}, 0, h->scal, scale, 1, h->ub_s, 0, N, h->stream, h->sink, h->lz_state);
+    launch_basis_combine(h->psi_s, lz_basis(h), h->n_pad, BasisCoef{}, 0, h->scal, scale, 1, h->ub_s, 0, N, h->stream, h->sink, h->lz_state);
     h->tail_done = h->sink.on;
     h->info.lanczos_matvecs = done; h->info.lanczos_exchanges = 0;
     if (m_io) *m_io = h->sc_host[LZ_HOST_SEQ] > 0.0 && h->sc_host[LZ_HOST_M] >= 1.0 ? (int)h->sc_host[LZ_HOST_M] : m_in;
@@ -866,11 +883,12 @@
     int pending_beta = 0;
     LzState st{0, 0, 0, 0, 1.0, {}, {}};
     bool hook_done = false;
+    bool y_from_list = false;
     auto update = [&](int j, bool scalars_only) {
         for (pse_handle *h : act(T)) {
             int rg[3][2];
             const int nrg = scalars_only ? 0 : update_ranges(h, N, rg);
-            launch_lz_update(lz_vec(h, j), h->w_s, lz_vec(h, j - 1), lz_vec(h, j + 1), j, h->scal, rg, nrg, h->stream, h->sums_all, T.G > 1 ? T.G : 0,
+            launch_lz_update(lz_vec(h, j), lz_y(h, y_from_list), lz_vec(h, j - 1), lz_vec(h, j + 1), j, h->scal, rg, nrg, h->stream, h->sums_all, T.G > 1 ? T.G : 0,
                              h == h0 ? h->sc_host_dev : nullptr, nullptr, T.G <= 1 ? vq_of(h) : nullptr, T.G <= 1 ? h->lz_sums : nullptr);
         }
     };
@@ -879,21 +897,25 @@
             const bool have_y = done == 0 && h0->w_is_mpsi;
             const bool fused = !have_y && h0->nb.cap > 0 && h0->nb_valid;
             const bool timed = done == 1 && fused;
-            if (!fused && !have_y) TRY(real(T, done == 0 ? &pse_handle::psi_s : &pse_handle::V, &pse_handle::w_s, (size_t)done * h0->n_pad, 0, N, true));
+            if (!fused && !have_y) {
+                TRY(lz_real_ok(h0, done));
+                TRY(real(T, done == 0 ? &pse_handle::psi_s : &pse_handle::V, &pse_handle::w_s, (size_t)done * h0->n_pad, 0, N, true));
+            }
+            y_from_list = fused;
             for (pse_handle *h : act(T)) {
                 int lo, hi;
                 row_range(h, N, lo, hi);
-                const double4 *xj = lz_vec(h, done), *vjm1 = lz_vec(h, done - 1);
+                const double4 *vjm1 = lz_vec4(h, done - 1);
                 if (fused) {
                     const bool ev = timed && h->timing;
                     const bool split = done > 0 && T.G <= 1;
-                    launch_mreal_lanczos(h->pos_s, xj, h->w_s, row_map(lo, hi), h->cell_off, h->dbox, h->nc, h->d.rcut, h->d.self, h->coef,
+                    launch_mreal_lanczos(h->pos_s, lz_vec(h, done), lz_y(h, true), row_map(lo, hi), h->cell_off, h->dbox, h->nc, h->d.rcut, h->d.self, h->coef,
                                          h->nb, LzFuse{split ? nullptr : vjm1, h->partials, h->npart_cap, nullptr, nullptr, nullptr, h->lz_sums, lz_update_grid(N)}, h->scal,
                                          ev ? h->ph[PH_MATVEC].a : nullptr, ev ? h->ph[PH_MATVEC].b : nullptr, h->stream,
                                          h->vl_use ? h->vl : VerletList{}, split ? 4 : 1, nullptr, DevRowArgs{}, done > 0 && T.G <= 1 ? vq_of(h) : nullptr);
                     if (timed) h->matvec_timed = true;
                 } else if (!(done == 0 && h->sums0_done)) {
-                    launch_lz_dots(xj, h->w_s, vjm1, lo, hi, h->partials, h->npart_cap, h->scal, h->stream);
+                    launch_lz_dots(lz_vec4(h, done), h->w_s, vjm1, lo, hi, h->partials, h->npart_cap, h->scal, h->stream);
                 }
                 h->w_is_mpsi = false; h->sums0_done = false;
             }
@@ -946,7 +968,7 @@
             const int j = done;
             const bool full = target - done >= 2 && j + 2 <= M_MAX;
             for (pse_handle *h : act(T)) {
-                const LzFuse lz{nullptr, h->partials, h->npart_cap, lz_vec(h, j), lz_vec(h, j - 1), j > 0 ? h->u_s : nullptr};
+                const LzFuse lz{nullptr, h->partials, h->npart_cap, lz_vec4(h, j), lz_vec4(h, j - 1), j > 0 ? h->u_s : nullptr};
                 if (j == 0 && !h->w_is_mpsi) return fail(PSE_ERR_NUMERIC, "two-step Lanczos: M psi did not come with the pair list");
                 if (!(j == 0 && h->w_is_mpsi)) {
                     launch_mreal_lanczos(h->pos_s, lz_vec(h, j), h->w_s, rank_rows(h, N, full ? 1 : 0), h->cell_off, h->dbox, h->nc, h->d.rcut,
@@ -1187,7 +1209,7 @@
     if (target + 2 * extra_blocks > M_MAX || !lz_decide_supported(target + 2 * extra_blocks))
         return fail(PSE_ERR_INVALID, "owned-particle step: starting count %d of the Lanczos iteration is beyond what the device-side decision takes", m_in);
     int n_exchanges = 0, matvecs = 0, done = 0, half_pending = -1;
-    auto fuse = [&](pse_handle *h, int j) { return LzFuse{nullptr, h->partials, h->npart_cap, lz_vec(h, j), lz_vec(h, j - 1), j > 0 ? h->u_s : nullptr}; };
+    auto fuse = [&](pse_handle *h, int j) { return LzFuse{nullptr, h->partials, h->npart_cap, lz_vec4(h, j), lz_vec4(h, j - 1), j > 0 ? h->u_s : nullptr}; };
     auto exchange = [&](bool full) -> int {
         if (pump) TRY(pump->upto(n_exchanges));
         ++n_exchanges;
@@ -1494,7 +1516,6 @@
     HIPCHK(hipSetDevice(h->device));
     if (h->n_slabs != 1 || !h->nb_valid || h->nb.cap <= 0 || h->sorted_N <= 0)
         return fail(PSE_ERR_INVALID, "pse_debug_matvec_ms: needs the pair list of a Brownian call on a single-GPU engine (call it right after one)");
-    const size_t stride = h->n_pad;
     const int N = h->sorted_N;
     RowMap rm{};
     rm.n = 1; rm.lo[0] = 0; rm.hi[0] = N;
@@ -1502,7 +1523,7 @@
     HIPCHK(hipEventCreate(&e0)); HIPCHK(hipEventCreate(&e1));
     auto run = [&](int n) {
         for (int r = 0; r < n; ++r)
-            launch_mreal_lanczos(h->pos_s, h->V + stride, h->w_s, rm, h->cell_off, h->dbox, h->nc, h->d.rcut, h->d.self, h->coef, h->nb,
+            launch_mreal_lanczos(h->pos_s, lz_vec(h, 1), lz_y(h, true), rm, h->cell_off, h->dbox, h->nc, h->d.rcut, h->d.self, h->coef, h->nb,
                                  LzFuse{h->psi_s, h->partials, h->npart_cap, nullptr, nullptr, nullptr}, h->scal, nullptr, nullptr, h->stream,
                                  VerletList{}, 1, nullptr, DevRowArgs{}, vq_of(h), true);
     };
diff --git a/pse_amd/csrc/pse_device.h b/pse_amd/csrc/pse_device.h
--- a/pse_amd/csrc/pse_device.h
+++ b/pse_amd/csrc/pse_device.h
@@ -99,6 +99,36 @@
     if ((threadIdx.x & 63) == 0) sh[w] = v;
     __syncthreads();
     return sh[0] + sh[1] + sh[2] + sh[3];
+}
+struct VecOut {
+    double *p; int packed;
+    VecOut() = default;
+    __host__ __device__ VecOut(double4 *a) : p(reinterpret_cast<double *>(a)), packed(0) {}
+    __host__ __device__ VecOut(double *a, int pk) : p(a), packed(pk) {}
+};
+struct VecIn {
+    const double *p; int packed;
+    VecIn() = default;
+    __host__ __device__ VecIn(const double4 *a) : p(reinterpret_cast<const double *>(a)), packed(0) {}
+    __host__ __device__ VecIn(const double *a, int pk) : p(a), packed(pk) {}
+    __host__ __device__ VecIn(const VecOut &v) : p(v.p), packed(v.packed) {}
+};
+__device__ __forceinline__ void row24_load(const double *__restrict__ a, size_t i, double &x, double &y, double &z) {
+    const double *r = a + 3 * i;
+    x = r[0]; y = r[1]; z = r[2];
+}
+__device__ __forceinline__ void row24_store(double *__restrict__ a, size_t i, double x, double y, double z) {
+    double *r = a + 3 * i;
+    r[0] = x; r[1] = y; r[2] = z;
+}
+__device__ __forceinline__ void row_load(const VecIn &v, size_t i, double &x, double &y, double &z) {
+    if (v.packed) { row24_load(v.p, i, x, y, z); return; }
+    const double4 q = reinterpret_cast<const double4 *>(v.p)[i];
+    x = q.x; y = q.y; z = q.z;
+}
+__device__ __forceinline__ void row_store(const VecOut &v, size_t i, double x, double y, double z) {
+    if (v.packed) { row24_store(v.p, i, x, y, z); return; }
+    reinterpret_cast<double4 *>(v.p)[i] = make_double4(x, y, z, 0.0);
 }
 __device__ __forceinline__ double reduce_partials(const double *partials, int n, double *sh) {
     double v = 0.0;
diff --git a/pse_amd/csrc/pse_engine.hip b/pse_amd/csrc/pse_engine.hip
--- a/pse_amd/csrc/pse_engine.hip
+++ b/pse_amd/csrc/pse_engine.hip
@@ -257,6 +257,7 @@
         t.place_trials = std::max(0, std::min(12, ienv("PSE_PLACE_TRIALS", 10)));
         t.vq = ienv("PSE_VQ", 1);
         if (const char *v = getenv("PSE_LANCZOS_OP")) t.lz_op = !strcmp(v, "fp64") ? PSE_LANCZOS_FP64 : PSE_LANCZOS_RECORDS16;
+        t.rows24 = ienv("PSE_ROWS24", 1);
         if (const char *v = getenv("PSE_TEAM_SCHED")) {
             int a = 1, b = 2, c = 3;
             if (sscanf(v, "%d,%d,%d", &a, &b, &c) == 3) { t.team_sched[0] = a; t.team_sched[1] = b; t.team_sched[2] = c; }
@@ -431,7 +432,11 @@
     if (h->tun.place_trials > 1 && h->own_z && h->own_y && h->grid_slabs == 1)
         TRY(place_grids(h, (size_t)(G.nxl + G.hl + G.nhalo) * G.Ny * G.Nz, (size_t)G.nxl * G.Ny * G.Nzp));
 
-    TRY(dmalloc(h, &h->V, (size_t)(M_MAX + 1) * n));
+    h->rows24 = h->n_slabs == 1 && !h->loc.on && h->nb.cap > 0 && h->tun.lz_op != PSE_LANCZOS_FP64 && h->tun.rows24 != 0;
+    if (h->rows24) {
+        TRY(dmalloc(h, &h->V, ((size_t)(M_MAX + 1) * n * 3 + 3) / 4));
+        h->w24 = reinterpret_cast<double *>(h->V);
+    } else TRY(dmalloc(h, &h->V, (size_t)(M_MAX + 1) * n));
     if (h->n_slabs == 1 && !h->loc.on && h->tun.vq > 0) TRY(dmalloc(h, (char **)&h->vq, (size_t)16 * n));
     TRY(dmalloc(h, &h->pv_rows, pair_virial_rows((int)n)));
     TRY(dmalloc(h, &h->scal, (size_t)LZ_NSCAL));
diff --git a/pse_amd/csrc/pse_handle.h b/pse_amd/csrc/pse_handle.h
--- a/pse_amd/csrc/pse_handle.h
+++ b/pse_amd/csrc/pse_handle.h
@@ -165,6 +165,7 @@
         int place_trials = 10;
         int lz_extra = 2;
         int lz_op = PSE_LANCZOS_RECORDS16;
+        int rows24 = 1;
     } tun;
     DCells bidx_nc = {0, 0, 0};
     hipEvent_t ev_fork = nullptr, ev_join = nullptr;
@@ -246,6 +247,8 @@
     void *fft_work = nullptr;
     size_t fft_work_bytes = 0;
     double4 *V = nullptr;
+    bool rows24 = false;
+    double *w24 = nullptr;
     double *scal = nullptr, *partials = nullptr;
     double *lz_sums = nullptr;
     double *sc_host = nullptr;
diff --git a/pse_amd/csrc/pse_kernels.h b/pse_amd/csrc/pse_kernels.h
--- a/pse_amd/csrc/pse_kernels.h
+++ b/pse_amd/csrc/pse_kernels.h
@@ -133,7 +133,7 @@
                   Gate gate = Gate{},
                   DevRowArgs dr = DevRowArgs{});
 bool mreal_table_in_lds(int ncoef);
-void launch_mreal_lanczos(const double4 *pos_s, const double4 *vec_s, double4 *w, RowMap rows, const int *cell_off,
+void launch_mreal_lanczos(const double4 *pos_s, VecIn vec, VecOut out, RowMap rows, const int *cell_off,
                           DBox box, DCells nc, double rcut, double self, const double *coef, NbList nb, LzFuse lz,
                           double *scal, hipEvent_t ev_begin, hipEvent_t ev_end, hipStream_t s,
                           VerletList vl = VerletList{},
diff --git a/pse_amd/csrc/pse_kernels.hip b/pse_amd/csrc/pse_kernels.hip
--- a/pse_amd/csrc/pse_kernels.hip
+++ b/pse_amd/csrc/pse_kernels.hip
@@ -606,8 +606,10 @@
 k_mreal_list(const double4 *__restrict__ pos_s, const double4 *__restrict__ vec_s, double4 *__restrict__ out_s, RowMap rm_arg,
              DBox box, double self, NbList nb, LzFuse lz,
              const int *__restrict__ cell_off, DCells nc, double rcut2, const double *__restrict__ coef, VerletList vl,
-             const int *__restrict__ stop, DevRowArgs dr, const vq4 *__restrict__ vec_q = nullptr) {
+             const int *__restrict__ stop, DevRowArgs dr, const vq4 *__restrict__ vec_q = nullptr, int packed = 0) {
     if (stop && *stop) return;
+    const VecIn vin{reinterpret_cast<const double *>(vec_s), packed & 1};
+    const VecOut vout{reinterpret_cast<double *>(out_s), (packed >> 1) & 1};
     const RowMapRegs rm(rm_arg, dr.rm);
     int nb_live = gridDim.x;
     if (dr.rm) {
@@ -628,7 +630,7 @@
     double ux = 0.0, uy = 0.0, uz = 0.0;
     double4 vi = make_double4(0.0, 0.0, 0.0, 0.0);
     if (active) {
-        vi = vec_s[i];
+        row_load(vin, i, vi.x, vi.y, vi.z);
         const int cnt = nb.cnt[i];
         if (cnt >= 0) {
             if (wv == 0) { ux = self * vi.x; uy = self * vi.y; uz = self * vi.z; }
@@ -653,6 +655,7 @@
 #pragma unroll
                 for (int u = 0; u < UNROLL; ++u) {
                     if (VQ && !F64) { vq[u] = vec_q[e[u] & JMASK]; continue; }
+                    if (vin.packed) { row24_load(vin.p, e[u] & JMASK, vxy[u].x, vxy[u].y, vz[u]); continue; }
                     const double4 *vj = vec_s + (e[u] & JMASK);
                     vxy[u] = *reinterpret_cast<const double2 *>(vj);
                     vz[u] = vj->z;
@@ -685,7 +688,8 @@
                 if (r2 < rcut2 && r2 > 0.0) {
                     double f, h;
                     eval_fg_lean(r2, coef, f, h);
-                    const double4 Fj = vec_s[j];
+                    double3 Fj;
+                    row_load(vin, j, Fj.x, Fj.y, Fj.z);
                     if (F64) pair_apply64(pair_coef64(f, h, dx, dy, dz), Fj.x, Fj.y, Fj.z, ux, uy, uz);
                     else pair_apply(pair_coef(f, h, dx, dy, dz), Fj.x, Fj.y, Fj.z, ux, uy, uz);
                 }
@@ -705,7 +709,8 @@
                     if (r2 < rcut2 && j != i && r2 > 0.0) {
                         double f, h;
                         eval_fg_lean(r2, coef, f, h);
-                        const double4 Fj = vec_s[j];
+                        double3 Fj;
+                        row_load(vin, j, Fj.x, Fj.y, Fj.z);
                         if (F64) pair_apply64(pair_coef64(f, h, dx, dy, dz), Fj.x, Fj.y, Fj.z, ux, uy, uz);
                         else pair_apply(pair_coef(f, h, dx, dy, dz), Fj.x, Fj.y, Fj.z, ux, uy, uz);
                     }
@@ -767,7 +772,7 @@
         }
     }
     if (active) {
-        out_s[i] = make_double4(ux, uy, uz, 0.0);
+        row_store(vout, i, ux, uy, uz);
         if (dr.stage_hi) {
             const int lb = dr.lr->last_begin, no = dr.lr->n_own;
             if (i >= lb && i < no && i - lb < dr.stage_cap) dr.stage_hi[i - lb] = make_double4(ux, uy, uz, 0.0);
@@ -835,23 +840,26 @@
 }
 
 int mreal_partials_needed(int rows) { return nblocks(std::max(rows, 1), 64); }
-void launch_mreal_lanczos(const double4 *pos_s, const double4 *vec_s, double4 *w, RowMap rm, const int *cell_off,
+void launch_mreal_lanczos(const double4 *pos_s, VecIn vec, VecOut out, RowMap rm, const int *cell_off,
                           DBox box, DCells nc, double rcut, double self, const double *coef, NbList nb, LzFuse lz,
                           double *scal, hipEvent_t ev_begin, hipEvent_t ev_end, hipStream_t s, VerletList vl,
                           int sums, const int *stop, DevRowArgs dr, const void *vec_q, bool no_reduce) {
+    const double4 *vec_s = reinterpret_cast<const double4 *>(vec.p);
+    double4 *w = reinterpret_cast<double4 *>(out.p);
+    const int packed = (vec.packed ? 1 : 0) | (out.packed ? 2 : 0);
     const int rows = std::max(dr.rm ? dr.rows_cap : rm.list_rows(), 1);
     if (ev_begin) (void)hipEventRecord(ev_begin, s);
     const int nb64 = nblocks(rows, 64);
-#define PSE_LIST(F) hipLaunchKernelGGL((k_mreal_list<F, 4, 256, 4>), dim3(nb64), dim3(256), 0, s, pos_s, vec_s, w, rm, box, self, nb, lz, cell_off, nc, rcut * rcut, coef, vl, stop, dr)
-#define PSE_LIST64(F) hipLaunchKernelGGL((k_mreal_list<F, 4, 256, 4, false, true>), dim3(nb64), dim3(256), 0, s, pos_s, vec_s, w, rm, box, self, nb, lz, cell_off, nc, rcut * rcut, coef, vl, stop, dr, nullptr)
+#define PSE_LIST(F) hipLaunchKernelGGL((k_mreal_list<F, 4, 256, 4>), dim3(nb64), dim3(256), 0, s, pos_s, vec_s, w, rm, box, self, nb, lz, cell_off, nc, rcut * rcut, coef, vl, stop, dr, nullptr, packed)
+#define PSE_LIST64(F) hipLaunchKernelGGL((k_mreal_list<F, 4, 256, 4, false, true>), dim3(nb64), dim3(256), 0, s, pos_s, vec_s, w, rm, box, self, nb, lz, cell_off, nc, rcut * rcut, coef, vl, stop, dr, nullptr, packed)
     if (nb.c64) {
         if (sums == 0) PSE_LIST64(0); else if (sums == 1) PSE_LIST64(1); else if (sums == 2) PSE_LIST64(2); else if (sums == 3) PSE_LIST64(3); else PSE_LIST64(4);
     } else if (sums == 1 && vec_q)
         hipLaunchKernelGGL((k_mreal_list<1, 4, 256, 4, true>), dim3(nb64), dim3(256), 0, s, pos_s, vec_s, w, rm, box, self, nb, lz, cell_off, nc, rcut * rcut, coef, vl, stop, dr,
-                           (const vq4 *)vec_q);
+                           (const vq4 *)vec_q, packed);
     else if (sums == 4 && vec_q)
         hipLaunchKernelGGL((k_mreal_list<4, 4, 256, 4, true>), dim3(nb64), dim3(256), 0, s, pos_s, vec_s, w, rm, box, self, nb, lz, cell_off, nc, rcut * rcut, coef, vl, stop, dr,
-                           (const vq4 *)vec_q);
+                           (const vq4 *)vec_q, packed);
     else if (sums == 0) PSE_LIST(0); else if (sums == 1) PSE_LIST(1); else if (sums == 2) PSE_LIST(2); else if (sums == 3) PSE_LIST(3); else PSE_LIST(4);
 #undef PSE_LIST64
 #undef PSE_LIST
diff --git a/pse_amd/csrc/pse_vectors.h b/pse_amd/csrc/pse_vectors.h
--- a/pse_amd/csrc/pse_vectors.h
+++ b/pse_amd/csrc/pse_vectors.h
@@ -11,7 +11,7 @@
 void launch_lz_reduce(const double *partials, int npart, int cap, int nsum, double *scal, const int *stop, hipStream_t s);
 struct BasisCoef { double t[104]; };
 struct CombineSink { bool on; const double4 *add_a, *add_b; const unsigned *tag_s; double4 *vel; double4 *rows; };
-void launch_basis_combine(const double4 *x0, const double4 *V, size_t stride, const BasisCoef &t, int m, const double *scal,
+void launch_basis_combine(VecIn x0, VecIn V, size_t stride, const BasisCoef &t, int m, const double *scal,
                           double scale, int use_norm, double4 *out_s, int lo, int hi, hipStream_t s, CombineSink sink = CombineSink{},
                           const struct LzState *st = nullptr);
 void launch_lz_dots(const double4 *x, const double4 *y, const double4 *vprev, int lo, int hi, double *partials, int cap,
@@ -29,7 +29,7 @@
 void launch_vq_roundtrip(const double *in, double *out, int n, hipStream_t s);
 int lz_update_grid(int rows);
 void launch_lz_reduce_split(const double *xy, int n_xy, const double *upd, int n_upd, double *scal, const int *stop, hipStream_t s);
-void launch_lz_update(const double4 *xin, const double4 *y, const double4 *xprev, double4 *xnext, int j,
+void launch_lz_update(VecIn xin, VecIn y, VecIn xprev, VecOut xnext, int j,
                       double *scal, const int (*row_ranges)[2], int n_ranges, hipStream_t s,
                       const double *sums_all = nullptr, int nranks = 0, double *sch = nullptr, const int *stop = nullptr,
                       void *xq = nullptr,
diff --git a/pse_amd/csrc/pse_vectors.hip b/pse_amd/csrc/pse_vectors.hip
--- a/pse_amd/csrc/pse_vectors.hip
+++ b/pse_amd/csrc/pse_vectors.hip
@@ -62,8 +62,7 @@
     hipLaunchKernelGGL(k_lz_reduce, dim3(3), dim3(1024), 0, s, xy, n_xy, 0, 3, scal, stop, upd, n_upd);
 }
 __global__ void __launch_bounds__(TPB)
-k_lz_update(const double4 *__restrict__ xin, const double4 *__restrict__ y, const double4 *__restrict__ xprev,
-            double4 *__restrict__ xnext, int j, double *__restrict__ scal, RowRanges rg,
+k_lz_update(VecIn xin, VecIn y, VecIn xprev, VecOut xnext, int j, double *__restrict__ scal, RowRanges rg,
             const double *__restrict__ sums_all, int nranks, double *__restrict__ sch, const int *__restrict__ stop, vq4 *__restrict__ xq,
             double *__restrict__ next_sums) {
     if (stop && *stop) return;
@@ -88,10 +87,11 @@
     double nn = 0.0, np = 0.0;
     for (int t = blockIdx.x * TPB + threadIdx.x; t < n0 + n1 + n2; t += gridDim.x * TPB) {
         const int i = t < n0 ? rg.lo[0] + t : (t < n0 + n1 ? rg.lo[1] + (t - n0) : rg.lo[2] + (t - n0 - n1));
-        const double4 p = xin[i], q = y[i];
+        double3 p, q;
+        row_load(xin, i, p.x, p.y, p.z); row_load(y, i, q.x, q.y, q.z);
         double nx = (q.x - alpha * p.x) * inv, ny = (q.y - alpha * p.y) * inv, nz = (q.z - alpha * p.z) * inv;
-        if (xprev) { const double4 m = xprev[i]; nx -= cp * m.x; ny -= cp * m.y; nz -= cp * m.z; }
-        xnext[i] = make_double4(nx, ny, nz, 0.0);
+        if (xprev.p) { double3 m; row_load(xprev, i, m.x, m.y, m.z); nx -= cp * m.x; ny -= cp * m.y; nz -= cp * m.z; }
+        row_store(xnext, i, nx, ny, nz);
         if (xq) xq[i] = vq_pack(nx, ny, nz);
         nn += nx * nx + ny * ny + nz * nz;
         np += nx * p.x + ny * p.y + nz * p.z;
@@ -355,7 +355,7 @@
     hipLaunchKernelGGL(k_lz_dots, dim3(g), dim3(TPB), 0, s, x, y, vprev, lo, hi, partials, cap);
     launch_lz_reduce(partials, g, cap, y ? 3 : 1, scal, nullptr, s);
 }
-void launch_lz_update(const double4 *xin, const double4 *y, const double4 *xprev, double4 *xnext, int j,
+void launch_lz_update(VecIn xin, VecIn y, VecIn xprev, VecOut xnext, int j,
                       double *scal, const int (*rg)[2], int nrg, hipStream_t s, const double *sums_all, int nranks, double *sch,
                       const int *stop, void *xq, double *next_sums) {
     RowRanges r{};
@@ -399,7 +399,7 @@
 }
 
 __global__ void __launch_bounds__(TPB)
-k_basis_combine(const double4 *__restrict__ x0, const double4 *__restrict__ V, size_t stride, BasisCoef tc, int m,
+k_basis_combine(VecIn x0, VecIn V, size_t stride, BasisCoef tc, int m,
                 const double *__restrict__ scal, double scale, int use_norm, double4 *__restrict__ out, int lo, int N, CombineSink sink,
                 const LzState *__restrict__ st) {
     const double *t = tc.t;
@@ -408,7 +408,8 @@
     for (int i = lo + blockIdx.x * TPB + threadIdx.x; i < N; i += gridDim.x * TPB) {
         double x = 0, y = 0, z = 0;
         for (int q = 0; q < m; ++q) {
-            const double4 v = q == 0 ? x0[i] : V[(size_t)q * stride + i];
+            double3 v;
+            if (q == 0) row_load(x0, i, v.x, v.y, v.z); else row_load(V, (size_t)q * stride + i, v.x, v.y, v.z);
             const double tq = t[q];
             x += tq * v.x; y += tq * v.y; z += tq * v.z;
         }
@@ -423,7 +424,7 @@
         else sink.rows[i] = make_double4(sx, sy, sz, (double)idx);
     }
 }
-void launch_basis_combine(const double4 *x0, const double4 *V, size_t stride, const BasisCoef &t_dev, int m, const double *scal,
+void launch_basis_combine(VecIn x0, VecIn V, size_t stride, const BasisCoef &t_dev, int m, const double *scal,
                           double scale, int use_norm, double4 *out_s, int lo, int hi, hipStream_t s, CombineSink sink, const LzState *st) {
     hipLaunchKernelGGL(k_basis_combine, dim3(std::min(2048, std::max(1, nblocks(hi - lo, TPB)))), dim3(TPB), 0, s, x0, V, stride,
                        t_dev, m, scal, scale, use_norm, out_s, lo, hi, sink, st);
```

New measurement: 338.7 million particle-steps/s, median of 6. +1.3%, better.
